# gradslam/gradslam

Hardware: AMD Instinct MI355X
Metric: frames/sec PointFusion 640x480 RGB-D (higher is better)
Workload: dtype f32

## Files before the change

### gradslam_amd/csrc/gs_assoc_dev.h

```cpp
#pragma once
#include "gs_common.h"

struct GsCamera {
  float Ri[9];
  float ti[3];
  float K[12];
};

GS_DEV GsCamera gs_camera(const float* __restrict__ pose16, const float* __restrict__ K16) {
  GsCamera c;
#pragma unroll
  for (int j = 0; j < 3; ++j)
#pragma unroll
    for (int k = 0; k < 3; ++k) c.Ri[3 * j + k] = pose16[4 * k + j];
  const float t0 = pose16[3], t1 = pose16[7], t2 = pose16[11];
#pragma unroll
  for (int j = 0; j < 3; ++j)
    c.ti[j] = gs_dot3_plain(-c.Ri[3 * j], -c.Ri[3 * j + 1], -c.Ri[3 * j + 2], t0, t1, t2);
#pragma unroll
  for (int i = 0; i < 12; ++i) c.K[i] = K16[i];
  return c;
}

GS_DEV bool gs_project_point_hw_q(const GsCamera& c, float p0, float p1, float p2, int H, int W, float u_hi, float v_hi,
                                  int& h_out, int& w_out, float* q) {
  const float q0 = gs_dot3_fma(p0, p1, p2, c.Ri[0], c.Ri[1], c.Ri[2]) + c.ti[0];
  const float q1 = gs_dot3_fma(p0, p1, p2, c.Ri[3], c.Ri[4], c.Ri[5]) + c.ti[1];
  const float q2 = gs_dot3_fma(p0, p1, p2, c.Ri[6], c.Ri[7], c.Ri[8]) + c.ti[2];
  q[0] = q0;
  q[1] = q1;
  q[2] = q2;
  const bool front = q2 > 0.0f;
  float r[3];
#pragma unroll
  for (int j = 0; j < 3; ++j) {
    float acc = c.K[4 * j] * q0;
    acc = acc + c.K[4 * j + 1] * q1;
    acc = acc + c.K[4 * j + 2] * q2;
    acc = acc + c.K[4 * j + 3] * 1.0f;
    r[j] = acc;
  }
  const float zz = (r[2] != 0.0f) ? r[2] : 1.0f;
  const float u = r[0] / zz, v = r[1] / zz;
  const bool in_frame = (u > -1e-3f) && (u < u_hi) && (v > -1e-3f) && (v < v_hi) && front;
  if (!in_frame) return false;
  int wi = (int)__builtin_rintf(u), hi = (int)__builtin_rintf(v);
  wi = wi < 0 ? 0 : (wi > W - 1 ? W - 1 : wi);
  hi = hi < 0 ? 0 : (hi > H - 1 ? H - 1 : hi);
  h_out = hi;
  w_out = wi;
  return true;
}
GS_DEV bool gs_project_point_hw(const GsCamera& c, float p0, float p1, float p2, int H, int W, float u_hi, float v_hi,
                                int& h_out, int& w_out) {
  float q[3];
  return gs_project_point_hw_q(c, p0, p1, p2, H, W, u_hi, v_hi, h_out, w_out, q);
}

GS_DEV int32_t gs_project_point(const GsCamera& c, float p0, float p1, float p2, int H, int W,
                                float u_hi, float v_hi) {
  int h, w;
  return gs_project_point_hw(c, p0, p1, p2, H, W, u_hi, v_hi, h, w) ? (int32_t)(h * W + w) : -1;
}

GS_DEV bool gs_on_lattice(int h, int w, int ds) {
  if ((ds & (ds - 1)) == 0) return ((h | w) & (ds - 1)) == 0;
  return ((unsigned)h % (unsigned)ds == 0u) && ((unsigned)w % (unsigned)ds == 0u);
}

GS_DEV bool gs_is_similar(const float* __restrict__ points, const float* __restrict__ normals,
                          const float* __restrict__ gvertex, const float* __restrict__ gnormal,
                          int64_t n, int64_t p, float dist_th, float dot_th) {
  const float f0 = gvertex[3 * p], f1 = gvertex[3 * p + 1], f2 = gvertex[3 * p + 2];
  const float q0 = points[3 * n], q1 = points[3 * n + 1], q2 = points[3 * n + 2];
  const float dist = gs_norm3(f0 - q0, f1 - q1, f2 - q2);
  const float dot = gs_dot3_plain(gnormal[3 * p], gnormal[3 * p + 1], gnormal[3 * p + 2], normals[3 * n],
                                  normals[3 * n + 1], normals[3 * n + 2]);
  return (dist < dist_th) && (dot > dot_th);
}

GS_DEV bool gs_is_similar_v(const float* __restrict__ points, const float* __restrict__ normals, const float* f,
                            const float* g, int64_t n, float dist_th, float dot_th) {
  const float q0 = points[3 * n], q1 = points[3 * n + 1], q2 = points[3 * n + 2];
  const float dist = gs_norm3(f[0] - q0, f[1] - q1, f[2] - q2);
  const float dot = gs_dot3_plain(g[0], g[1], g[2], normals[3 * n], normals[3 * n + 1], normals[3 * n + 2]);
  return (dist < dist_th) && (dot > dot_th);
}

GS_DEV uint64_t gs_assoc_key(const float* __restrict__ points, const float* __restrict__ ccounts,
                             const float* __restrict__ gvertex, int64_t n, int64_t p) {
  const float inv = 1.0f / (ccounts[n] + 1e-20f);
  const float d0 = points[3 * n] - gvertex[3 * p];
  const float d1 = points[3 * n + 1] - gvertex[3 * p + 1];
  const float d2 = points[3 * n + 2] - gvertex[3 * p + 2];
  float ray = d0 * d0 + d1 * d1;
  ray = ray + d2 * d2;
  return ((uint64_t)__float_as_uint(inv) << 32) | (uint64_t)__float_as_uint(ray);
}
GS_DEV uint64_t gs_assoc_key_v(const float* __restrict__ points, const float* __restrict__ ccounts, const float* f,
                               int64_t n) {
  const float inv = 1.0f / (ccounts[n] + 1e-20f);
  const float d0 = points[3 * n] - f[0];
  const float d1 = points[3 * n + 1] - f[1];
  const float d2 = points[3 * n + 2] - f[2];
  float ray = d0 * d0 + d1 * d1;
  ray = ray + d2 * d2;
  return ((uint64_t)__float_as_uint(inv) << 32) | (uint64_t)__float_as_uint(ray);
}
```

### gradslam_amd/csrc/gs_fuse.hip

```cpp
#include "gs_assoc_dev.h"
#include "gs_compact.h"

__global__ void __launch_bounds__(256) gs_fuse_init_kernel(int32_t* __restrict__ pix_of, int64_t n,
                                                           int32_t* __restrict__ any_flag) {
  const int64_t i = (int64_t)blockIdx.x * 256 + threadIdx.x;
  if (i == 0) *any_flag = 0;
  if (i < n) pix_of[i] = -1;
}

__global__ void __launch_bounds__(256) gs_fuse_scatter_kernel(const int32_t* __restrict__ best_pix,
                                                              int64_t P, GsCount n_map_c,
                                                              int32_t* __restrict__ pix_of,
                                                              int32_t* __restrict__ any_flag) {
  const int64_t p = (int64_t)blockIdx.x * 256 + threadIdx.x;
  if (p >= P) return;
  const int32_t n = best_pix[p];
  if (n >= 0 && n < gs_count(n_map_c)) {
    pix_of[n] = (int32_t)p;
    *any_flag = 1;
  }
}

struct FrameGlobalMaps {
  const float* __restrict__ gvertex;
  const float* __restrict__ gnormal;
  __device__ void operator()(const int64_t p, float* fp, float* fn) const {
#pragma unroll
    for (int k = 0; k < 3; ++k) {
      fp[k] = gvertex[3 * p + k];
      fn[k] = gnormal[3 * p + k];
    }
  }
  __device__ void vertex_of(const int64_t p, float* fp) const {
#pragma unroll
    for (int k = 0; k < 3; ++k) fp[k] = gvertex[3 * p + k];
  }
  __device__ void normal_of(const int64_t p, float* fn) const {
#pragma unroll
    for (int k = 0; k < 3; ++k) fn[k] = gnormal[3 * p + k];
  }
};
struct FrameLocalMaps {
  const float* __restrict__ vertex;
  const float* __restrict__ normal;
  float T[12];
  __device__ void operator()(const int64_t p, float* fp, float* fn) const {
    float v[3], n[3];
#pragma unroll
    for (int k = 0; k < 3; ++k) {
      v[k] = vertex[3 * p + k];
      n[k] = normal[3 * p + k];
    }
    const float validf = v[2] > 0.0f ? 1.0f : 0.0f;
    float g0, g1, g2;
    gs_rigid_fma(T, v[0], v[1], v[2], g0, g1, g2);
    fp[0] = g0 * validf; fp[1] = g1 * validf; fp[2] = g2 * validf;
    fn[0] = gs_dot3_fma(T[0], T[1], T[2], n[0], n[1], n[2]);
    fn[1] = gs_dot3_fma(T[4], T[5], T[6], n[0], n[1], n[2]);
    fn[2] = gs_dot3_fma(T[8], T[9], T[10], n[0], n[1], n[2]);
  }
  __device__ void vertex_of(const int64_t p, float* fp) const {
    float v[3];
#pragma unroll
    for (int k = 0; k < 3; ++k) v[k] = vertex[3 * p + k];
    const float validf = v[2] > 0.0f ? 1.0f : 0.0f;
    float g0, g1, g2;
    gs_rigid_fma(T, v[0], v[1], v[2], g0, g1, g2);
    fp[0] = g0 * validf; fp[1] = g1 * validf; fp[2] = g2 * validf;
  }
  __device__ void normal_of(const int64_t p, float* fn) const {
    float n[3];
#pragma unroll
    for (int k = 0; k < 3; ++k) n[k] = normal[3 * p + k];
    fn[0] = gs_dot3_fma(T[0], T[1], T[2], n[0], n[1], n[2]);
    fn[1] = gs_dot3_fma(T[4], T[5], T[6], n[0], n[1], n[2]);
    fn[2] = gs_dot3_fma(T[8], T[9], T[10], n[0], n[1], n[2]);
  }
};
GS_DEV FrameLocalMaps frame_local_maps(const float* vertex, const float* normal, const float* pose16) {
  FrameLocalMaps f;
  f.vertex = vertex; f.normal = normal;
#pragma unroll
  for (int i = 0; i < 12; ++i) f.T[i] = pose16[i];
  return f;
}

template <class Frame>
GS_DEV void fuse_merge_row(float* __restrict__ points, float* __restrict__ normals, float* __restrict__ colors,
                           float* __restrict__ ccounts, const int64_t n, const int32_t p, const Frame& frame,
                           const float* __restrict__ rgb, const float* __restrict__ alpha) {
  const float a = p >= 0 ? alpha[p] : 0.0f;
  const float cc = ccounts[n];
  float P[3], N[3], C[3], fp[3] = {0.0f, 0.0f, 0.0f}, fn[3] = {0.0f, 0.0f, 0.0f}, fc[3] = {0.0f, 0.0f, 0.0f};
#pragma unroll
  for (int k = 0; k < 3; ++k) {
    P[k] = points[3 * n + k];
    N[k] = normals[3 * n + k];
    C[k] = colors[3 * n + k];
  }
  if (p >= 0) {
    frame((int64_t)p, fp, fn);
#pragma unroll
    for (int k = 0; k < 3; ++k) fc[k] = rgb[3 * (int64_t)p + k];
  }
  const float cc2 = cc + a;
  const float inv = 1.0f / (cc2 == 0.0f ? 1.0f : cc2);
#pragma unroll
  for (int k = 0; k < 3; ++k) {
    P[k] = ((cc * P[k]) + (a * fp[k])) * inv;
    N[k] = ((cc * N[k]) + (a * fn[k])) * inv;
    C[k] = ((cc * C[k]) + (a * fc[k])) * inv;
  }
#pragma unroll
  for (int k = 0; k < 3; ++k) points[3 * n + k] = P[k];
#pragma unroll
  for (int k = 0; k < 3; ++k) normals[3 * n + k] = N[k];
#pragma unroll
  for (int k = 0; k < 3; ++k) colors[3 * n + k] = C[k];
  ccounts[n] = cc2;
}

__global__ void __launch_bounds__(256) gs_fuse_merge_kernel(
    float* __restrict__ points, float* __restrict__ normals, float* __restrict__ colors,
    float* __restrict__ ccounts, GsCount n_map_c, const int32_t* __restrict__ pix_of,
    const int32_t* __restrict__ any_flag, const float* __restrict__ gvertex,
    const float* __restrict__ gnormal, const float* __restrict__ rgb, const float* __restrict__ alpha,
    int renorm_all) {
  const int64_t n = (int64_t)blockIdx.x * 256 + threadIdx.x;
  if (n >= gs_count(n_map_c)) return;
  if (*any_flag == 0 && renorm_all != 2) return;
  const int32_t p = pix_of[n];
  if (p < 0 && !renorm_all) return;
  fuse_merge_row(points, normals, colors, ccounts, n, p, FrameGlobalMaps{gvertex, gnormal}, rgb, alpha);
}

struct PredNewPixel {
  const float* depth;
  const int32_t* best_pix;
  __device__ bool operator()(int64_t p) const {
    return depth[p] > 0.0f && (best_pix == nullptr || best_pix[p] < 0);
  }
};
template <class Frame>
struct EmitAppendT {
  float* points;
  float* normals;
  float* colors;
  float* ccounts;
  GsCount n_map;
  Frame frame;
  const float* rgb;
  const float* alpha;
  __device__ void operator()(int64_t p, int64_t pos) const {
    const int64_t r = gs_count(n_map) + pos;
    float v[3], nn[3] = {0.0f, 0.0f, 0.0f}, c[3] = {0.0f, 0.0f, 0.0f};
    frame.vertex_of(p, v);
    if (normals) frame.normal_of(p, nn);
    if (colors) {
#pragma unroll
      for (int k = 0; k < 3; ++k) c[k] = rgb[3 * p + k];
    }
    const float a = ccounts ? alpha[p] : 0.0f;
#pragma unroll
    for (int k = 0; k < 3; ++k) points[3 * r + k] = v[k];
    if (normals) {
#pragma unroll
      for (int k = 0; k < 3; ++k) normals[3 * r + k] = nn[k];
    }
    if (colors) {
#pragma unroll
      for (int k = 0; k < 3; ++k) colors[3 * r + k] = c[k];
    }
    if (ccounts) ccounts[r] = a;
  }
};
typedef EmitAppendT<FrameGlobalMaps> EmitAppend;

static int fuse_append(float* points, float* normals, float* colors, float* ccounts, GsCount n_map_c,
                       int64_t capacity, const int32_t* best_pix, const float* gvertex, const float* gnormal,
                       const float* rgb, const float* alpha, const float* depth, int H, int W, int renorm_all,
                       int64_t* new_count_out, void* scratch, void* stream) {
  const int64_t n_map_host = n_map_c.host;
  GS_REQUIRE(H > 0 && W > 0 && n_map_host >= 0 && capacity >= n_map_host, "bad sizes");
  GS_REQUIRE(points && normals && colors && ccounts && best_pix && gvertex && gnormal && rgb && alpha &&
                 depth && new_count_out && scratch,
             "NULL pointer");
  hipStream_t st = gs_stream(stream);
  const int64_t P = (int64_t)H * W;
  const int64_t n_map = n_map_host;
  char* base = reinterpret_cast<char*>(scratch) + gs_cp_scratch_bytes(P > n_map ? P : n_map);
  int32_t* any_flag = reinterpret_cast<int32_t*>(base);
  int32_t* pix_of = reinterpret_cast<int32_t*>(base + 256);
  GsProf prof(GS_PROF_FUSE, 88.0 * (double)n_map + 45.0 * (double)P, st);
  if (n_map > 0) {
    hipLaunchKernelGGL(gs_fuse_init_kernel, dim3((unsigned)gs_ceil_div(n_map, 256)), dim3(256), 0, st,
                       pix_of, n_map, any_flag);
    hipLaunchKernelGGL(gs_fuse_scatter_kernel, dim3((unsigned)gs_ceil_div(P, 256)), dim3(256), 0, st,
                       best_pix, P, n_map_c, pix_of, any_flag);
    hipLaunchKernelGGL(gs_fuse_merge_kernel, dim3((unsigned)gs_ceil_div(n_map, 256)), dim3(256), 0, st,
                       points, normals, colors, ccounts, n_map_c, pix_of, any_flag, gvertex, gnormal, rgb,
                       alpha, renorm_all);
    GS_LAUNCH_CHECK();
  }
  EmitAppend emit{points, normals, colors, ccounts, n_map_c, FrameGlobalMaps{gvertex, gnormal}, rgb, alpha};
  return gs_compact(GsCount{P, nullptr}, PredNewPixel{depth, best_pix}, emit, new_count_out, n_map_c, capacity,
                    scratch, st);
}

extern "C" int gs_fuse_append_f32(float* points, float* normals, float* colors, float* ccounts,
                                  int64_t n_map_host, int64_t capacity, const int32_t* best_pix,
                                  const float* gvertex, const float* gnormal, const float* rgb,
                                  const float* alpha, const float* depth, int H, int W, int renorm_all,
                                  int64_t* new_count_out, void* scratch, void* stream) {
  return fuse_append(points, normals, colors, ccounts, GsCount{n_map_host, nullptr}, capacity, best_pix, gvertex,
                     gnormal, rgb, alpha, depth, H, W, renorm_all, new_count_out, scratch, stream);
}
extern "C" int gs_fuse_append_dc_f32(float* points, float* normals, float* colors, float* ccounts,
                                     int64_t n_map_bound, const int64_t* n_map_dev, int64_t capacity,
                                     const int32_t* best_pix, const float* gvertex, const float* gnormal,
                                     const float* rgb, const float* alpha, const float* depth, int H, int W,
                                     int renorm_all, int64_t* new_count_out, void* scratch, void* stream) {
  GS_REQUIRE(n_map_dev && capacity >= n_map_bound + (int64_t)H * W, "device-count fuse needs capacity >= bound + H*W");
  return fuse_append(points, normals, colors, ccounts, GsCount{n_map_bound, n_map_dev}, capacity, best_pix,
                     gvertex, gnormal, rgb, alpha, depth, H, W, renorm_all, new_count_out, scratch, stream);
}

static int append_valid(float* points, float* normals, float* colors, float* ccounts, GsCount n_map_c,
                        int64_t capacity, const float* gvertex, const float* gnormal, const float* rgb,
                        const float* alpha, const float* depth, int H, int W, int64_t* new_count_out,
                        void* scratch, void* stream) {
  GS_REQUIRE(H > 0 && W > 0 && n_map_c.host >= 0 && capacity >= n_map_c.host, "bad sizes");
  GS_REQUIRE(points && gvertex && depth && new_count_out && scratch, "NULL pointer");
  EmitAppend emit{points, gnormal ? normals : nullptr, rgb ? colors : nullptr, alpha ? ccounts : nullptr,
                  n_map_c, FrameGlobalMaps{gvertex, gnormal}, rgb, alpha};
  return gs_compact(GsCount{(int64_t)H * W, nullptr}, PredNewPixel{depth, nullptr}, emit, new_count_out, n_map_c,
                    capacity, scratch, gs_stream(stream));
}
extern "C" int gs_append_valid_f32(float* points, float* normals, float* colors, float* ccounts,
                                   int64_t n_map_host, int64_t capacity, const float* gvertex,
                                   const float* gnormal, const float* rgb, const float* alpha,
                                   const float* depth, int H, int W, int64_t* new_count_out,
                                   void* scratch, void* stream) {
  return append_valid(points, normals, colors, ccounts, GsCount{n_map_host, nullptr}, capacity, gvertex, gnormal,
                      rgb, alpha, depth, H, W, new_count_out, scratch, stream);
}
extern "C" int gs_append_valid_dc_f32(float* points, float* normals, float* colors, float* ccounts,
                                      int64_t n_map_bound, const int64_t* n_map_dev, int64_t capacity,
                                      const float* gvertex, const float* gnormal, const float* rgb,
                                      const float* alpha, const float* depth, int H, int W,
                                      int64_t* new_count_out, void* scratch, void* stream) {
  GS_REQUIRE(n_map_dev && capacity >= n_map_bound + (int64_t)H * W, "device-count append needs capacity >= bound + H*W");
  return append_valid(points, normals, colors, ccounts, GsCount{n_map_bound, n_map_dev}, capacity, gvertex,
                      gnormal, rgb, alpha, depth, H, W, new_count_out, scratch, stream);
}

__global__ void __launch_bounds__(256) gs_fuse_bwd_rows_kernel(
    const float* __restrict__ points, const float* __restrict__ normals, const float* __restrict__ colors,
    const float* __restrict__ ccounts, int64_t n_old, const int32_t* __restrict__ pix_of,
    const int32_t* __restrict__ any_flag, const float* __restrict__ gvertex, const float* __restrict__ gnormal,
    const float* __restrict__ rgb, const float* __restrict__ alpha, int renorm_all,
    const float* __restrict__ P_bar, const float* __restrict__ N_bar, const float* __restrict__ C_bar,
    const float* __restrict__ F_bar, float* __restrict__ oP_bar, float* __restrict__ oN_bar,
    float* __restrict__ oC_bar, float* __restrict__ oF_bar, float* __restrict__ gv_bar, float* __restrict__ gn_bar,
    float* __restrict__ rgb_bar, float* __restrict__ alpha_bar) {
  const int64_t n = (int64_t)blockIdx.x * 256 + threadIdx.x;
  if (n >= n_old) return;
  const int32_t p = (*any_flag != 0) ? pix_of[n] : -1;
  if ((*any_flag == 0 && renorm_all != 2) || (p < 0 && !renorm_all)) {
#pragma unroll
    for (int k = 0; k < 3; ++k) {
      oP_bar[3 * n + k] = P_bar[3 * n + k];
      oN_bar[3 * n + k] = N_bar[3 * n + k];
      oC_bar[3 * n + k] = C_bar[3 * n + k];
    }
    oF_bar[n] = F_bar[n];
    return;
  }
  const double a = p >= 0 ? (double)alpha[p] : 0.0;
  const double cc = (double)ccounts[n];
  const double cc2 = cc + a;
  const double inv = 1.0 / (cc2 == 0.0 ? 1.0 : cc2);
  double inv_bar = 0.0, cc_bar = 0.0, a_bar = 0.0;
  const float* olds[3] = {points, normals, colors};
  const float* frames[3] = {gvertex, gnormal, rgb};
  const float* bars[3] = {P_bar, N_bar, C_bar};
  float* obars[3] = {oP_bar, oN_bar, oC_bar};
  float* fbars[3] = {gv_bar, gn_bar, rgb_bar};
#pragma unroll
  for (int t = 0; t < 3; ++t) {
#pragma unroll
    for (int k = 0; k < 3; ++k) {
      const double x = (double)olds[t][3 * n + k];
      const double f = p >= 0 ? (double)frames[t][3 * (int64_t)p + k] : 0.0;
      const double xb = (double)bars[t][3 * n + k];
      const double ub = xb * inv;
      inv_bar += xb * (cc * x + a * f);
      obars[t][3 * n + k] = (float)(cc * ub);
      if (p >= 0) fbars[t][3 * (int64_t)p + k] = (float)(a * ub);
      cc_bar += x * ub;
      a_bar += f * ub;
    }
  }
  const double cc2_bar = (double)F_bar[n] + (cc2 != 0.0 ? -inv * inv * inv_bar : 0.0);
  oF_bar[n] = (float)(cc_bar + cc2_bar);
  if (p >= 0) alpha_bar[p] = (float)(a_bar + cc2_bar);
}

struct EmitAppendBackward {
  const float* P_bar;
  const float* N_bar;
  const float* C_bar;
  const float* F_bar;
  int64_t n_old;
  float* gv_bar;
  float* gn_bar;
  float* rgb_bar;
  float* alpha_bar;
  __device__ void operator()(int64_t p, int64_t pos) const {
    const int64_t r = n_old + pos;
#pragma unroll
    for (int k = 0; k < 3; ++k) {
      gv_bar[3 * p + k] = P_bar[3 * r + k];
      gn_bar[3 * p + k] = N_bar[3 * r + k];
      rgb_bar[3 * p + k] = C_bar[3 * r + k];
    }
    alpha_bar[p] = F_bar[r];
  }
};

extern "C" int gs_fuse_append_backward_f32(const float* points, const float* normals, const float* colors,
                                           const float* ccounts, int64_t n_old, const int32_t* best_pix,
                                           const float* gvertex, const float* gnormal, const float* rgb,
                                           const float* alpha, const float* depth, int H, int W, int renorm_all,
                                           const float* P_bar, const float* N_bar, const float* C_bar,
                                           const float* F_bar, int64_t n_new, float* old_points_bar,
                                           float* old_normals_bar, float* old_colors_bar, float* old_ccounts_bar,
                                           float* gvertex_bar, float* gnormal_bar, float* rgb_bar, float* alpha_bar,
                                           void* scratch, void* stream) {
  GS_REQUIRE(H > 0 && W > 0 && n_old >= 0 && n_new >= n_old, "bad sizes");
  GS_REQUIRE(best_pix && gvertex && gnormal && rgb && alpha && depth && P_bar && N_bar && C_bar && F_bar && gvertex_bar &&
                 gnormal_bar && rgb_bar && alpha_bar && scratch,
             "NULL pointer");
  hipStream_t st = gs_stream(stream);
  const int64_t P = (int64_t)H * W;
  GS_HIP(hipMemsetAsync(gvertex_bar, 0, 12 * (size_t)P, st));
  GS_HIP(hipMemsetAsync(gnormal_bar, 0, 12 * (size_t)P, st));
  GS_HIP(hipMemsetAsync(rgb_bar, 0, 12 * (size_t)P, st));
  GS_HIP(hipMemsetAsync(alpha_bar, 0, 4 * (size_t)P, st));
  char* base = reinterpret_cast<char*>(scratch) + gs_cp_scratch_bytes(P > n_old ? P : n_old);
  int32_t* any_flag = reinterpret_cast<int32_t*>(base);
  int32_t* pix_of = reinterpret_cast<int32_t*>(base + 256);
  if (n_old > 0) {
    GS_REQUIRE(points && normals && colors && ccounts && old_points_bar && old_normals_bar && old_colors_bar &&
                   old_ccounts_bar,
               "NULL pointer");
    const GsCount n_old_c{n_old, nullptr};
    hipLaunchKernelGGL(gs_fuse_init_kernel, dim3((unsigned)gs_ceil_div(n_old, 256)), dim3(256), 0, st, pix_of, n_old,
                       any_flag);
    hipLaunchKernelGGL(gs_fuse_scatter_kernel, dim3((unsigned)gs_ceil_div(P, 256)), dim3(256), 0, st, best_pix, P,
                       n_old_c, pix_of, any_flag);
    hipLaunchKernelGGL(gs_fuse_bwd_rows_kernel, dim3((unsigned)gs_ceil_div(n_old, 256)), dim3(256), 0, st, points,
                       normals, colors, ccounts, n_old, pix_of, any_flag, gvertex, gnormal, rgb, alpha, renorm_all, P_bar,
                       N_bar, C_bar, F_bar, old_points_bar, old_normals_bar, old_colors_bar, old_ccounts_bar,
                       gvertex_bar, gnormal_bar, rgb_bar, alpha_bar);
    GS_LAUNCH_CHECK();
  }
  EmitAppendBackward emit{P_bar, N_bar, C_bar, F_bar, n_old, gvertex_bar, gnormal_bar, rgb_bar, alpha_bar};
  int64_t* cnt = reinterpret_cast<int64_t*>(base + 128);
  return gs_compact(P, PredNewPixel{depth, best_pix}, emit, cnt, 0, n_new - n_old, scratch, st);
}

constexpr int32_t MU_TIE_MARK = 0x7fffffff;
struct MuSeq {
  float* points; float* normals; float* colors; float* ccounts;
  GsCount n_map;
  int64_t capacity;
  const float* vertex; const float* normal; const float* depth; const float* rgb; const float* alpha;
  const float* pose16; const float* K16;
  float* gvertex; float* gnormal;
  int32_t* best_pix;
  int64_t* new_count_out;
  int32_t* any_flag;
  uint64_t* key_pix;
  int32_t* tile_counts;
  uint64_t* key_pt;
  int32_t* pix;
  int32_t* pix_of;
};
struct MuBatch {
  int B, H, W, renorm_all;
  int64_t P, ntiles;
  float u_hi, v_hi, dist_th, dot_th;
  int32_t* call_flag;
  int zero_call_flag;
  MuSeq s[GS_MAX_BATCH];
};

__global__ void __launch_bounds__(256) gs_mu_pixel_init_kernel(const MuBatch mb) {
  const MuSeq& q = mb.s[blockIdx.x % mb.B];
  const int64_t p = (int64_t)(blockIdx.x / mb.B) * 256 + threadIdx.x;
  if (p == 0) { q.any_flag[0] = 0; q.any_flag[1] = 0; }
  if (blockIdx.x == 0 && threadIdx.x == 0 && mb.zero_call_flag) *mb.call_flag = 0;
  if (p >= mb.P) return;
  float T[12];
#pragma unroll
  for (int i = 0; i < 12; ++i) T[i] = q.pose16[i];
  const float validf = q.depth[p] > 0.0f ? 1.0f : 0.0f;
  float g0, g1, g2;
  gs_rigid_fma(T, q.vertex[3 * p], q.vertex[3 * p + 1], q.vertex[3 * p + 2], g0, g1, g2);
  q.gvertex[3 * p] = g0 * validf;
  q.gvertex[3 * p + 1] = g1 * validf;
  q.gvertex[3 * p + 2] = g2 * validf;
  const float n0 = q.normal[3 * p], n1 = q.normal[3 * p + 1], n2 = q.normal[3 * p + 2];
  q.gnormal[3 * p] = gs_dot3_fma(T[0], T[1], T[2], n0, n1, n2);
  q.gnormal[3 * p + 1] = gs_dot3_fma(T[4], T[5], T[6], n0, n1, n2);
  q.gnormal[3 * p + 2] = gs_dot3_fma(T[8], T[9], T[10], n0, n1, n2);
  q.key_pix[p] = ~0ull;
  q.best_pix[p] = -1;
}

__global__ void __launch_bounds__(256) gs_mu_project_key_kernel(const MuBatch mb) {
  const MuSeq& q = mb.s[blockIdx.x % mb.B];
  const int64_t n = (int64_t)(blockIdx.x / mb.B) * 256 + threadIdx.x;
  if (n >= gs_count(q.n_map)) return;
  const GsCamera c = gs_camera(q.pose16, q.K16);
  const int32_t p = gs_project_point(c, q.points[3 * n], q.points[3 * n + 1], q.points[3 * n + 2], mb.H, mb.W, mb.u_hi,
                                     mb.v_hi);
  int32_t pk = -1;
  if (p >= 0) {
    float fp[3], fn[3];
    if (q.gvertex) FrameGlobalMaps{q.gvertex, q.gnormal}((int64_t)p, fp, fn);
    else frame_local_maps(q.vertex, q.normal, q.pose16)((int64_t)p, fp, fn);
    if (gs_is_similar_v(q.points, q.normals, fp, fn, n, mb.dist_th, mb.dot_th)) {
      const uint64_t k = gs_assoc_key_v(q.points, q.ccounts, fp, n);
      const unsigned long long old = atomicMin(reinterpret_cast<unsigned long long*>(&q.key_pix[p]), (unsigned long long)k);
      if (old == (unsigned long long)k) {
        q.best_pix[p] = MU_TIE_MARK;
        q.any_flag[1] = 1;
      }
      q.key_pt[n] = k;
      pk = p;
    }
  }
  q.pix[n] = pk;
}

GS_DEV void mu_settle_ties(const MuSeq& q, const unsigned blk, const unsigned nblk) {
  if (q.any_flag[1] == 0) return;
  const int64_t n_map = gs_count(q.n_map);
  for (int64_t n = (int64_t)blk * GS_CP_BLOCK + threadIdx.x; n < n_map; n += (int64_t)nblk * GS_CP_BLOCK) {
    const int32_t p = q.pix[n];
    if (p < 0 || q.best_pix[p] == -1) continue;
    if (q.key_pt[n] == q.key_pix[p]) atomicMin(reinterpret_cast<unsigned*>(&q.best_pix[p]), (unsigned)n);
  }
}

__global__ void __launch_bounds__(GS_CP_BLOCK) gs_mu_winner_count_kernel(const MuBatch mb) {
  __shared__ int smem[GS_CP_BLOCK / GS_WAVE + 1];
  const MuSeq& q = mb.s[blockIdx.x % mb.B];
  const unsigned blk = blockIdx.x / mb.B;
  const int64_t base = (int64_t)blk * GS_CP_TILE + (int64_t)threadIdx.x * GS_CP_ITEMS;
  int c = 0;
  uint64_t kk[GS_CP_ITEMS];
  float dd[GS_CP_ITEMS];
#pragma unroll
  for (int i = 0; i < GS_CP_ITEMS; ++i) {
    const int64_t pc = base + i < mb.P ? base + i : mb.P - 1;
    kk[i] = q.key_pix[pc];
    dd[i] = q.depth[pc];
  }
  bool any = false;
#pragma unroll
  for (int i = 0; i < GS_CP_ITEMS; ++i) {
    const int64_t p = base + i;
    if (p < mb.P) {
      const bool matched = kk[i] != ~0ull;
      any = any || matched;
      if (dd[i] > 0.0f && !matched) ++c;
    }
  }
  if (any) {
    q.any_flag[0] = 1;
    *mb.call_flag = 1;
  }
  int total;
  (void)gs_block_excl_scan<GS_CP_BLOCK>(c, smem, &total);
  if (threadIdx.x == 0) q.tile_counts[blk] = total;
  mu_settle_ties(q, blk, gridDim.x / mb.B);
}

GS_DEV void mu_merge_body(const MuBatch& mb, const unsigned bid) {
  const MuSeq& q = mb.s[bid % mb.B];
  const int64_t n = (int64_t)(bid / mb.B) * 256 + threadIdx.x;
  if (n >= gs_count(q.n_map)) return;
  if (*mb.call_flag == 0) return;
  int32_t p = q.pix[n];
  if (p >= 0) {
    bool win = q.key_pt[n] == q.key_pix[p];
    if (win) {
      const int32_t bp = q.best_pix[p];
      win = bp == -1 || bp == (int32_t)n;
      if (win && bp == -1) q.best_pix[p] = (int32_t)n;
    }
    if (!win) p = -1;
  }
  if (p < 0 && !mb.renorm_all) return;
  if (q.gvertex) fuse_merge_row(q.points, q.normals, q.colors, q.ccounts, n, p, FrameGlobalMaps{q.gvertex, q.gnormal}, q.rgb, q.alpha);
  else fuse_merge_row(q.points, q.normals, q.colors, q.ccounts, n, p, frame_local_maps(q.vertex, q.normal, q.pose16), q.rgb, q.alpha);
}

GS_DEV void mu_append_body(const MuBatch& mb, const unsigned bid) {
  __shared__ int smem[GS_CP_BLOCK / GS_WAVE + 1];
  const MuSeq& q = mb.s[bid % mb.B];
  const unsigned blk = bid / mb.B;
  int before = 0, all = 0;
  for (int64_t t = threadIdx.x; t < mb.ntiles; t += GS_CP_BLOCK) {
    const int v = q.tile_counts[t];
    all += v;
    if (t < (int64_t)blk) before += v;
  }
  int tile_prefix, total_new, tile_new;
  (void)gs_block_excl_scan<GS_CP_BLOCK>(before, smem, &tile_prefix);
  (void)gs_block_excl_scan<GS_CP_BLOCK>(all, smem, &total_new);
  const int64_t n_map = gs_count(q.n_map);
  if (blk == 0 && threadIdx.x == 0) q.new_count_out[0] = n_map + total_new;
  const int64_t base = (int64_t)blk * GS_CP_TILE + (int64_t)threadIdx.x * GS_CP_ITEMS;
  bool keep[GS_CP_ITEMS];
  int c = 0;
  {
    uint64_t kk[GS_CP_ITEMS];
    float dd[GS_CP_ITEMS];
#pragma unroll
    for (int i = 0; i < GS_CP_ITEMS; ++i) {
      const int64_t pc = base + i < mb.P ? base + i : mb.P - 1;
      kk[i] = q.key_pix[pc];
      dd[i] = q.depth[pc];
    }
#pragma unroll
    for (int i = 0; i < GS_CP_ITEMS; ++i) {
      keep[i] = base + i < mb.P && dd[i] > 0.0f && kk[i] == ~0ull;
      c += keep[i] ? 1 : 0;
    }
  }
  int w = gs_block_excl_scan<GS_CP_BLOCK>(c, smem, &tile_new);
  __shared__ unsigned short loc_s[GS_CP_TILE];
#pragma unroll
  for (int i = 0; i < GS_CP_ITEMS; ++i) {
    if (keep[i]) loc_s[w++] = (unsigned short)(threadIdx.x * GS_CP_ITEMS + i);
  }
  __syncthreads();
  const int64_t tile_base = (int64_t)blk * GS_CP_TILE;
  if (q.gvertex) {
    const EmitAppend emit{q.points, q.normals, q.colors, q.ccounts, q.n_map, FrameGlobalMaps{q.gvertex, q.gnormal}, q.rgb, q.alpha};
    for (int r = threadIdx.x; r < tile_new; r += GS_CP_BLOCK) {
      const int64_t pos = (int64_t)tile_prefix + r;
      if (n_map + pos < q.capacity) emit(tile_base + loc_s[r], pos);
    }
  } else {
    const EmitAppendT<FrameLocalMaps> emit{q.points, q.normals, q.colors, q.ccounts, q.n_map,
                                           frame_local_maps(q.vertex, q.normal, q.pose16), q.rgb, q.alpha};
    for (int r = threadIdx.x; r < tile_new; r += GS_CP_BLOCK) {
      const int64_t pos = (int64_t)tile_prefix + r;
      if (n_map + pos < q.capacity) emit(tile_base + loc_s[r], pos);
    }
  }
}

static_assert(GS_CP_BLOCK == 256, "merge and append blocks share a launch");
__global__ void __launch_bounds__(256) gs_mu_merge_append_kernel(const MuBatch mb, const unsigned nb_append) {
  if (blockIdx.x < nb_append) mu_append_body(mb, blockIdx.x);
  else mu_merge_body(mb, blockIdx.x - nb_append);
}

extern "C" int64_t gs_update_map_scratch_bytes(int64_t n_map_bound, int H, int W) {
  const int64_t P = (int64_t)H * W;
  return (int64_t)(256 + gs_align(8 * (size_t)P) + gs_align(4 * (size_t)gs_cp_tiles(P)) +
                   gs_align(8 * (size_t)(n_map_bound > 0 ? n_map_bound : 1)) +
                   2 * gs_align(4 * (size_t)(n_map_bound > 0 ? n_map_bound : 1)) + 4096);
}

int32_t* gs_update_map_call_flag(void* scratch0) { return reinterpret_cast<int32_t*>(scratch0) + 32; }
void gs_update_map_tables(void* scratch, int32_t** any_flag, uint64_t** key_pix) {
  *any_flag = reinterpret_cast<int32_t*>(scratch);
  *key_pix = reinterpret_cast<uint64_t*>(reinterpret_cast<char*>(scratch) + 256);
}

static int update_chunk(const gs_update_seq* seqs, int B, int H, int W, float dist_th, float dot_th, int renorm_all,
                        hipStream_t st, int phase, int32_t* call_flag, bool first_chunk, bool tables_ready) {
  MuBatch mb;
  mb.B = B; mb.H = H; mb.W = W; mb.renorm_all = renorm_all;
  mb.call_flag = call_flag; mb.zero_call_flag = first_chunk ? 1 : 0;
  mb.P = (int64_t)H * W;
  mb.ntiles = gs_cp_tiles(mb.P);
  mb.u_hi = (float)((double)W - 0.999); mb.v_hi = (float)((double)H - 0.999);
  mb.dist_th = dist_th; mb.dot_th = dot_th;
  int64_t n_max = 0;
  double bytes_assoc = 0.0, bytes_fuse = 0.0;
  for (int b = 0; b < B; ++b) {
    const gs_update_seq& u = seqs[b];
    const int64_t n_map = u.map.n_bound;
    n_max = n_map > n_max ? n_map : n_max;
    char* q = reinterpret_cast<char*>(u.scratch);
    MuSeq& m = mb.s[b];
    m.points = u.map.points; m.normals = u.map.normals; m.colors = u.map.colors; m.ccounts = u.map.ccounts;
    m.n_map = GsCount{u.map.n_bound, u.map.n_dev};
    m.capacity = u.map.capacity;
    m.vertex = u.vertex; m.normal = u.normal; m.depth = u.depth; m.rgb = u.rgb; m.alpha = u.alpha;
    m.pose16 = u.pose16; m.K16 = u.K16;
    m.gvertex = u.gvertex; m.gnormal = u.gnormal; m.best_pix = u.best_pix; m.new_count_out = u.new_count_out;
    m.any_flag = reinterpret_cast<int32_t*>(q); q += 256;
    m.key_pix = reinterpret_cast<uint64_t*>(q); q += gs_align(8 * (size_t)mb.P);
    m.tile_counts = reinterpret_cast<int32_t*>(q); q += gs_align(4 * (size_t)mb.ntiles);
    m.key_pt = reinterpret_cast<uint64_t*>(q); q += gs_align(8 * (size_t)(n_map > 0 ? n_map : 1));
    m.pix = reinterpret_cast<int32_t*>(q); q += gs_align(4 * (size_t)(n_map > 0 ? n_map : 1));
    m.pix_of = reinterpret_cast<int32_t*>(q);
    bytes_assoc += 72.0 * (double)n_map;
    bytes_fuse += 104.0 * (double)n_map + 49.0 * (double)mb.P;
  }
  const unsigned uB = (unsigned)B;
  const unsigned pb = uB * (unsigned)gs_ceil_div(mb.P, 256), nb = uB * (unsigned)gs_ceil_div(n_max > 0 ? n_max : 1, 256);
  if (phase == 0) {
    if (!tables_ready) {
      GsProf prof(GS_PROF_FRAME, (double)B * (double)mb.P * 64.0, st);
      hipLaunchKernelGGL(gs_mu_pixel_init_kernel, dim3(pb), dim3(256), 0, st, mb);
    }
    if (n_max > 0) {
      GsProf prof(GS_PROF_ASSOC, bytes_assoc, st, 1);
      hipLaunchKernelGGL(gs_mu_project_key_kernel, dim3(nb), dim3(256), 0, st, mb);
    }
    GsProf prof(GS_PROF_FUSE, bytes_fuse / 3.0, st, 1);
    hipLaunchKernelGGL(gs_mu_winner_count_kernel, dim3(uB * (unsigned)mb.ntiles), dim3(GS_CP_BLOCK), 0, st, mb);
  } else {
    GsProf prof(GS_PROF_FUSE, bytes_fuse * (2.0 / 3.0), st, 1);
    const unsigned nb_append = uB * (unsigned)mb.ntiles;
    hipLaunchKernelGGL(gs_mu_merge_append_kernel, dim3(nb_append + (n_max > 0 ? nb : 0u)), dim3(256), 0, st, mb, nb_append);
  }
  GS_LAUNCH_CHECK();
  return GS_OK;
}

int gs_update_map_fusion_batch_impl(const gs_update_seq* seqs_host, int B, int H, int W, float dist_th, float dot_th,
                                    int renorm_all, void* stream, bool tables_ready) {
  GS_REQUIRE(seqs_host && B > 0 && H > 0 && W > 0, "bad arguments");
  GS_REQUIRE((int64_t)H * W < (1ll << 31), "too large for int32 indices");
  for (int b = 0; b < B; ++b) {
    const gs_update_seq& u = seqs_host[b];
    GS_REQUIRE(u.map.n_bound >= 0 && u.map.n_bound < 0x7fffffff, "bad map size");
    GS_REQUIRE(u.map.capacity >= u.map.n_bound + (int64_t)H * W, "capacity must cover n_bound + H*W rows");
    GS_REQUIRE(u.map.points && u.map.normals && u.map.colors && u.map.ccounts && u.vertex && u.normal && u.depth && u.rgb &&
                   u.alpha && u.pose16 && u.K16 && u.best_pix && u.new_count_out && u.scratch,
               "NULL pointer");
    GS_REQUIRE((u.gvertex && u.gnormal) || (tables_ready && !u.gvertex && !u.gnormal), "gvertex / gnormal: both or none");
    GS_REQUIRE(u.new_count_out != u.map.n_dev, "new_count_out must not alias the map's device count");
  }
  hipStream_t st = gs_stream(stream);
  int32_t* call_flag = gs_update_map_call_flag(seqs_host[0].scratch);
  for (int phase = 0; phase < 2; ++phase) {
    for (int c0 = 0; c0 < B; c0 += GS_MAX_BATCH) {
      const int nb = B - c0 < GS_MAX_BATCH ? B - c0 : GS_MAX_BATCH;
      const int rc = update_chunk(seqs_host + c0, nb, H, W, dist_th, dot_th, renorm_all, st, phase, call_flag, c0 == 0,
                                  tables_ready);
      if (rc != GS_OK) return rc;
    }
  }
  return GS_OK;
}

extern "C" int gs_update_map_fusion_batch_f32(const gs_update_seq* seqs_host, int B, int H, int W, float dist_th,
                                              float dot_th, int renorm_all, void* stream) {
  return gs_update_map_fusion_batch_impl(seqs_host, B, H, W, dist_th, dot_th, renorm_all, stream, false);
}

extern "C" int gs_update_map_fusion_dc_f32(float* points, float* normals, float* colors, float* ccounts,
                                           int64_t n_map_bound, const int64_t* n_map_dev, int64_t capacity,
                                           const float* vertex, const float* normal, const float* depth,
                                           const float* rgb, const float* alpha, const float* pose16,
                                           const float* K16, int H, int W, float dist_th, float dot_th,
                                           int renorm_all, float* gvertex, float* gnormal, int32_t* best_pix,
                                           int64_t* new_count_out, void* scratch, void* stream) {
  gs_update_seq u;
  u.map = gs_map_view{points, normals, colors, ccounts, capacity, n_map_bound, n_map_dev};
  u.vertex = vertex; u.normal = normal; u.depth = depth; u.rgb = rgb; u.alpha = alpha;
  u.pose16 = pose16; u.K16 = K16;
  u.gvertex = gvertex; u.gnormal = gnormal; u.best_pix = best_pix; u.new_count_out = new_count_out; u.scratch = scratch;
  return gs_update_map_fusion_batch_f32(&u, 1, H, W, dist_th, dot_th, renorm_all, stream);
}
```

### gradslam_amd/csrc/gs_icp_loop.hip

```cpp
#include <stdlib.h>
#include <string.h>

#include <memory>
#include <mutex>
#include <optional>
#include <type_traits>

#include "gs_env.h"
#include "gs_icp_math.h"
#include "gs_knn.h"
#include "gs_knn_bbox.h"

constexpr int GS_ICP_MAX_ITERS = 1024;
struct GsIcpState {
  IcpSmall s[2];
  float trace[GS_ICP_MAX_ITERS * 12];
};

struct TapePtrs {
  float* src;
  int32_t* idx;
  float* sys;
};
GS_DEV void tape_write_sys(float* __restrict__ sys, int it, const double* S, float damp) {
// ... 873 lines not shown
    if (FULL && out_idx) out_idx[s] = j;
    if (tape_idx) tape_idx[s] = keep ? (int32_t)j : -1;
    if (keep) {
      if (FULL) {
        int q = 0;
#pragma unroll
        for (int i = 0; i < 6; ++i)
#pragma unroll
          for (int k = i; k < 6; ++k) v[q++] = (double)a[i] * (double)a[k];
#pragma unroll
        for (int i = 0; i < 6; ++i) v[21 + i] = (double)a[i] * (double)r;
      }
      v[27] = (double)r * (double)r;
    }
  }
  const int lane = threadIdx.x & 63, wave = threadIdx.x >> 6;
#pragma unroll
  for (int i = FULL ? 0 : 27; i < LIN_NV; ++i) {
    const double sum = gs_wave_sum_f64(v[i]);
    if (lane == 0) red[wave][i] = sum;
  }
  __syncthreads();
  if (threadIdx.x < LIN_NV && (FULL || threadIdx.x == 27)) {
    const int i = threadIdx.x;
    partials[(int64_t)blockIdx.x * LIN_NV + i] = ((red[0][i] + red[1][i]) + red[2][i]) + red[3][i];
  }
}

__global__ void __launch_bounds__(SUM_BLOCK) gs_icp_solve_kernel(const double* __restrict__ partials, int nrows,
                                                                 GsIcpState* __restrict__ st, int it,
                                                                 float* __restrict__ tape_sys) {
  __shared__ double S[32];
  __shared__ double sub[SUM_BLOCK / 32][32];
  __shared__ float xi_s[8];
  icp_sum_rows<SUM_BLOCK>(partials, nrows, S, sub);
  if (threadIdx.x >= GS_WAVE) return;
  gs_solve_spd6_wave(S, st->s[0].damp, xi_s);
  __builtin_amdgcn_wave_barrier();
  if (threadIdx.x != 0) return;
  IcpSmall sm = st->s[0];
  if (tape_sys) tape_write_sys(tape_sys, it, S, sm.damp);
  for (int k = 0; k < 6; ++k) sm.xi[k] = xi_s[k];
  icp_solve_finish(S, sm);
  st->s[0] = sm;
}

__global__ void __launch_bounds__(SUM_BLOCK) gs_icp_update_kernel(const double* __restrict__ partials, int nrows,
                                                                  GsIcpState* __restrict__ st, gs_icp_params prm,
                                                                  int it, const float* __restrict__ compose16,
                                                                  float* __restrict__ out_T16) {
  __shared__ double red[SUM_BLOCK / GS_WAVE];
  const double e1 = icp_sum_col27<SUM_BLOCK>(partials, nrows, red);
  if (threadIdx.x != 0) return;
  IcpSmall sm = st->s[0];
  icp_update_math((float)e1, sm, prm, it < GS_ICP_MAX_ITERS ? st->trace + 12 * it : nullptr);
  st->s[0] = sm;
  if (it == prm.numiters - 1) icp_write_result(sm, compose16, out_T16);
}

GS_DEV IcpSmall icp_state_init(const float* __restrict__ init16, float damp) {
  IcpSmall sm;
  for (int i = 0; i < 16; ++i) {
    sm.T_total[i] = init16[i];
    sm.T_step[i] = init16[i];
    sm.Tr[i] = (i % 5 == 0) ? 1.0f : 0.0f;
  }
  for (int i = 0; i < 8; ++i) sm.xi[i] = 0.0f;
  sm.damp = damp;
  sm.err = 0.0f;
  sm.pad[0] = sm.pad[1] = 0.0f;
  return sm;
}
__global__ void gs_icp_init_kernel(GsIcpState* __restrict__ st, const float* __restrict__ init16, float damp,
                                   int numiters, const float* __restrict__ compose16, float* __restrict__ out_T16) {
  if (threadIdx.x != 0) return;
  const IcpSmall sm = icp_state_init(init16, damp);
  st->s[0] = sm;
  st->s[1] = sm;
  if (numiters == 0) icp_write_result(sm, compose16, out_T16);
}

template <class T>
static T* gs_at(void* base, size_t offset) { return reinterpret_cast<T*>(reinterpret_cast<char*>(base) + offset); }
struct GsTake { size_t end = 0; size_t operator()(size_t n) { end += n; return end - n; } };

constexpr int ICP_ROWRED_DOUBLES = 32;
struct IcpLayout { size_t state, rowred, sync, best, srcA, srcB, partials[2], grid, total; };
static IcpLayout icp_layout(int64_t n_src, int64_t n_tgt) {
  GsTake take;
  IcpLayout L;
  L.state = take(gs_align(sizeof(GsIcpState)));
  L.rowred = take(gs_align(sizeof(double) * ICP_ROWRED_DOUBLES));
  L.sync = L.rowred + sizeof(double) * LIN_NV;
  static_assert(8 * ICP_ROWRED_DOUBLES >= 8 * LIN_NV + 4 * PS_WORDS, "the sync record does not fit behind rowred + LIN_NV");
  L.best = take(gs_align(8 * (size_t)n_src));
  L.srcA = take(gs_align(12 * (size_t)n_src)); L.srcB = take(gs_align(12 * (size_t)n_src));
  for (int k = 0; k < 2; ++k) L.partials[k] = take(gs_align(sizeof(double) * LIN_NV * icp_rows(n_src)));
  L.grid = take(gs_knn_grid_scratch_bytes(n_src, n_tgt));
  L.total = take.end + 4096;
  return L;
}
struct IcpScratch {
  GsIcpState* state;
  double* rowred;
  unsigned* sync;
  unsigned long long* best; float *srcA, *srcB;
  double* partials[2]; void* grid;
};
static IcpScratch icp_carve(void* p, const IcpLayout& L) {
  return IcpScratch{gs_at<GsIcpState>(p, L.state), gs_at<double>(p, L.rowred), gs_at<unsigned>(p, L.sync),
                    gs_at<unsigned long long>(p, L.best), gs_at<float>(p, L.srcA), gs_at<float>(p, L.srcB),
                    {gs_at<double>(p, L.partials[0]), gs_at<double>(p, L.partials[1])}, gs_at<void>(p, L.grid)};
}

extern "C" int64_t gs_icp_scratch_bytes(int64_t n_src, int64_t n_tgt) { return (int64_t)icp_layout(n_src < 1 ? 1 : n_src, n_tgt).total; }

static int icp_tape_finish(void* tape, const GsIcpState* state, int64_t n_src, int numiters, hipStream_t st) {
  GsIcpTape t = gs_icp_tape_carve(tape, n_src, numiters);
  if (numiters > 0)
    GS_HIP(hipMemcpyAsync(t.trace, state->trace, sizeof(float) * 12 * (size_t)numiters, hipMemcpyDeviceToDevice, st));
  return GS_OK;
}

static double icp_alg_bytes(int numiters, int64_t n_slots, int64_t n_queries, int64_t n_binned) {
  const double rows = (double)gs_ceil_div(n_slots, FS_QPB);
  const double full = 12.0 * n_slots + 36.0 * n_queries + 8.0 * LIN_NV * rows + 16.0 * n_binned;
  const double look = 12.0 * n_slots + 24.0 * n_queries + 8.0 * rows + 16.0 * n_binned;
  return (double)numiters * (full + look);
}

struct LocSeq {
  const float* vertex;
  const float* depth;
  const float* pose16;
  float* lattice;
  GsIcpState* state;
  float* out_pose16;
  char* clear_ptr;
  int64_t* n_valid;
  int* far_n;
  int* lstat;
  float4* wl_cq;
  unsigned* sync;
};
struct LocBatch {
  int B, W, ds, Wl;
  int64_t n_lat;
  size_t clear_bytes;
  float damp;
  int numiters;
  int count_valid;
  LocSeq s[GS_MAX_BATCH];
};
constexpr int LP_CLEAR_ITEMS = 8;

GS_DEV void loc_prep_block(const LocBatch& lb, const unsigned bid, const unsigned nb_lat) {
  const LocSeq& q = lb.s[bid % lb.B];
  const unsigned blk = bid / lb.B;
  if (blk < nb_lat) {
    const int64_t e = (int64_t)blk * 256 + threadIdx.x;
    int valid = 0;
    if (e < lb.n_lat) {
      const int64_t p = (e / lb.Wl) * lb.ds * (int64_t)lb.W + (e % lb.Wl) * lb.ds;
      float g0 = __builtin_nanf(""), g1 = g0, g2 = g0;
      if (q.depth[p] > 0.0f) {
        float T[12];
#pragma unroll
        for (int i = 0; i < 12; ++i) T[i] = q.pose16[i];
        gs_rigid_fma(T, q.vertex[3 * p], q.vertex[3 * p + 1], q.vertex[3 * p + 2], g0, g1, g2);
        valid = 1;
      }
      q.lattice[3 * e] = g0; q.lattice[3 * e + 1] = g1; q.lattice[3 * e + 2] = g2;
      if (q.wl_cq) q.wl_cq[e] = make_float4(0.0f, 0.0f, 0.0f, 0.0f);
    }
    const unsigned long long m = lb.count_valid ? __ballot(valid) : 0ull;
    if ((threadIdx.x & 63) == 0 && m) atomicAdd(reinterpret_cast<unsigned long long*>(q.n_valid), (unsigned long long)__popcll(m));
    if (blk == 0 && threadIdx.x == 0) {
      float id[16];
      for (int i = 0; i < 16; ++i) id[i] = (i % 5 == 0) ? 1.0f : 0.0f;
      const IcpSmall sm = icp_state_init(id, lb.damp);
      q.state->s[0] = sm;
      q.state->s[1] = sm;
      if (q.far_n)
        for (int i = 0; i < FS_FAR_PASSES; ++i) q.far_n[i] = 0;
      if (q.lstat)
        for (int i = 0; i < 3 * GL_STAT_LAUNCHES; ++i) q.lstat[i] = 0;
      if (q.sync)
        for (int i = 0; i < PS_WORDS; ++i) q.sync[i] = 0u;
      if (lb.numiters == 0) icp_write_result(sm, q.pose16, q.out_pose16);
    }
    return;
  }
  float4* dst = reinterpret_cast<float4*>(q.clear_ptr);
  const size_t n16 = lb.clear_bytes / 16;
  const size_t base = (size_t)(blk - nb_lat) * 256 * LP_CLEAR_ITEMS + threadIdx.x;
#pragma unroll
  for (int u = 0; u < LP_CLEAR_ITEMS; ++u) {
    const size_t i = base + (size_t)u * 256;
    if (i < n16) dst[i] = make_float4(0.0f, 0.0f, 0.0f, 0.0f);
  }
}
__global__ void __launch_bounds__(256) gs_loc_prep_kernel(const LocBatch lb, unsigned nb_lat) {
  loc_prep_block(lb, blockIdx.x, nb_lat);
}
static_assert(GB_BLOCK == 256, "lattice and bbox blocks share a launch");
__global__ void __launch_bounds__(256) gs_loc_prep_bbox_kernel(const LocBatch lb, const GsGridBatch gb, const unsigned nb_lat,
                                                               const float u_hi, const float v_hi) {
  const unsigned n_prep = (unsigned)lb.B * nb_lat;
  if (blockIdx.x < n_prep) loc_prep_block(lb, blockIdx.x, nb_lat);
  else gridb_bbox_block(gb, blockIdx.x - n_prep, u_hi, v_hi);
}

static int64_t loc_lattice(int H, int W, int ds) { return (int64_t)((H + ds - 1) / ds) * ((W + ds - 1) / ds); }

struct ListMem {
  float4* lq;
  uint32_t* ls;
  int* stat;
};

struct FarMem {
  uint32_t* c;
  float4* cq;
  int* idx;
  int* n;
};

struct FarBuildSeq {
  const float* src;
  const int* idx;
  const int* n;
  const GsGrid* gp;
  const int* cell_start;
  const float4* sorted;
  float* d2prev;
  FarMem m;
};
struct FarBuildBatch {
  int B;
  FarBuildSeq s[GS_MAX_BATCH];
};
constexpr int FAR_BLOCK = 512;
constexpr int FAR_BLOCKS_PER_SEQ = 64;
__global__ void __launch_bounds__(FAR_BLOCK) gs_icp_far_build_kernel(const FarBuildBatch fb) {
  const FarBuildSeq& q = fb.s[blockIdx.x % fb.B];
  const int blk = (int)(blockIdx.x / fb.B);
  const int n = *q.n;
  if (blk >= n) return;
  constexpr int NG = FAR_BLOCK / FS_HG;
  __shared__ float qs[NG][3];
  __shared__ float d1_s[NG];
  __shared__ uint8_t flag_s[NG];
  __shared__ int unres_q[NG], sq_s[NG];
  __shared__ int unres_n;
  __shared__ uint32_t stage_s[NG][GS_FAR_SLOTS + 4];
  const GsGrid g = *q.gp;
  const int grp = threadIdx.x / FS_HG, l16 = threadIdx.x & (FS_HG - 1);
  for (int base = blk; base < n; base += FAR_BLOCKS_PER_SEQ * NG) {
    if (threadIdx.x == 0) unres_n = 0;
    __syncthreads();
    const int e = base + grp * FAR_BLOCKS_PER_SEQ;
    if (e < n) {
      const int sq = q.idx[e];
      const float hx = q.src[3 * (int64_t)sq], hy = q.src[3 * (int64_t)sq + 1], hz = q.src[3 * (int64_t)sq + 2];
      const float4 found = q.m.cq[sq];
      const float d1 = sqrtf(found.x);
      const int kdone = (int)found.y;
      if (kdone >= 0) {
        const float R = far_emit_cube<FS_HG>(g, q.cell_start, q.sorted, hx, hy, hz, l16, d1, kdone, stage_s[grp],
                                             reinterpret_cast<int*>(&stage_s[grp][GS_FAR_SLOTS]));
        for (int u = l16; u < GS_FAR_SLOTS; u += FS_HG) q.m.c[GS_FAR_SLOTS * (int64_t)sq + u] = stage_s[grp][u];
        if (l16 == 0) {
          q.m.cq[sq] = make_float4(hx, hy, hz, R);
          if (R > 0.0f) q.d2prev[sq] = __uint_as_float(__float_as_uint(q.d2prev[sq]) | 0x80000000u);
        }
      } else if (l16 == 0) {
        qs[grp][0] = hx; qs[grp][1] = hy; qs[grp][2] = hz;
        d1_s[grp] = d1;
        sq_s[grp] = sq;
        unres_q[atomicAdd(&unres_n, 1)] = grp;
      }
    }
    __syncthreads();
    const int nun = unres_n;
    for (int u = 0; u < nun; u += FS_BQ) {
      const int nq = nun - u < FS_BQ ? nun - u : FS_BQ;
      block_brute_collect_multi<FAR_BLOCK, FS_BQ>(qs, unres_q + u, nq, q.sorted, q.cell_start[g.ncell], d1_s,
                                                  GS_FAR_RADD * g.c, sq_s, q.m.cq, q.m.c, flag_s);
      if ((int)threadIdx.x < nq) {
        const int gq = unres_q[u + threadIdx.x];
        const int s2 = sq_s[gq];
        if (flag_s[gq]) q.d2prev[s2] = __uint_as_float(__float_as_uint(q.d2prev[s2]) | 0x80000000u);
      }
    }
    __syncthreads();
  }
}

static int64_t loc_rows(const gs_map_view& m) { return m.capacity > m.n_bound ? m.capacity : m.n_bound; }

struct LocLayout {
  int64_t n_lat, rows;
  IcpLayout sc;
  size_t lattice, pix, n_valid, icp, lq, ls, lstat, far_c, far_cq, far_idx, far_n, far_out4, total;
};
static LocLayout loc_layout(int64_t n_lat, int64_t rows) {
  GsTake take;
  LocLayout L;
  L.n_lat = n_lat; L.rows = rows > 0 ? rows : 1;
  L.lattice = take(gs_align(12 * (size_t)n_lat));
  L.pix = take(gs_align(4 * (size_t)L.rows));
  L.n_valid = take(256);
  L.sc = icp_layout(n_lat, L.rows);
  L.icp = take(L.sc.total);
  L.lq = take(gs_align(16 * (size_t)n_lat));
  L.ls = take(gs_align(4 * GL_SLOTS * (size_t)n_lat));
  L.lstat = take(gs_align(4 * 3 * GL_STAT_LAUNCHES));
  L.far_c = take(gs_align(4 * GS_FAR_SLOTS * (size_t)n_lat));
  L.far_cq = take(gs_align(16 * (size_t)n_lat));
  L.far_idx = take(gs_align(4 * FS_FAR_PASSES * (size_t)n_lat));
  L.far_n = take(256);
  L.far_out4 = L.far_n + 4 * 8;
  static_assert(FS_FAR_PASSES <= 8, "the far-list counters run into the result words");
  L.total = take.end;
  return L;
}
static bool loc_lists_fit(const LocLayout& L) { return L.total - (L.icp + L.sc.partials[1]) >= sizeof(double) * LIN_NV * FS_BLOCK; }

extern "C" int64_t gs_localize_scratch_bytes(int H, int W, int ds, int64_t n_map_bound) {
  if (H < 1 || W < 1 || ds < 1) return 0;
  return (int64_t)loc_layout(loc_lattice(H, W, ds), n_map_bound).total;
}

struct LocCarve {
  float* lattice; int32_t* pix; int64_t* n_valid;
  IcpScratch sc; GridMem gm; ListMem lm;
  FarMem fm; int* far_out4;
};
static LocCarve loc_carve(void* p, const LocLayout& L) {
  const IcpScratch sc = icp_carve(gs_at<char>(p, L.icp), L.sc);
  return LocCarve{gs_at<float>(p, L.lattice), gs_at<int32_t>(p, L.pix), gs_at<int64_t>(p, L.n_valid), sc,
                  grid_carve(sc.grid, L.n_lat, L.rows),
                  ListMem{gs_at<float4>(p, L.lq), gs_at<uint32_t>(p, L.ls), gs_at<int>(p, L.lstat)},
                  FarMem{gs_at<uint32_t>(p, L.far_c), gs_at<float4>(p, L.far_cq), gs_at<int>(p, L.far_idx), gs_at<int>(p, L.far_n)},
                  gs_at<int>(p, L.far_out4)};
}
static LocCarve loc_carve_of(const void* scratch, int H, int W, int ds, int64_t map_rows) {
  return loc_carve(const_cast<void*>(scratch), loc_layout(loc_lattice(H, W, ds), map_rows));
}

struct IcpEnginePlan {
  bool far_on, wide_on, lists_on, persist_on;
  bool binned_normals;
  bool reduce_rows;
  int lists_from;
  IcpHalfPlan half;
  int ps_it0, ps_nb, ps_upb;
  float weak_room;
  int lmode(int it, bool look_ahead) const {
    if (!lists_on || it < lists_from) return 0;
    if (it > lists_from) return 2;
    return look_ahead ? (persist_on ? 3 : 1) : 0;
  }
};
static IcpEnginePlan icp_engine_plan(const GsEnv& env, const IcpDevice& dev, int B, int64_t n_lat, int numiters,
                                     const LocLayout* layouts) {
  IcpEnginePlan p;
  const int64_t rows = (int64_t)icp_rows(n_lat);
  p.binned_normals = env.icp_binned_normals; p.weak_room = env.icp_weak_room;
  p.lists_from = env.icp_lists_from >= 0 ? env.icp_lists_from : FS_LISTS_FROM;
  p.reduce_rows = rows > FS_REDUCE_ROWS;
  p.far_on = env.icp_far && numiters > 0;
  p.wide_on = env.icp_wide && !p.far_on && numiters > 0;
  p.ps_upb = (int)gs_ceil_div(rows, PS_CUS_PER_XCD);
  p.ps_nb = (int)gs_ceil_div(rows, p.ps_upb > 0 ? p.ps_upb : 1);
  const bool persist_asked = env.icp_persist && env.icp_lists && !p.far_on && B <= (int)GS_XCDS && p.ps_upb <= PS_UPB &&
                             numiters > p.lists_from + 1 && !env.icp_timeline && !env.icp_lanes_set && dev.ps_fits &&
                             p.binned_normals;
  p.half = icp_half_plan(env, dev.cus, n_lat, B, p.far_on ? 4 : (persist_asked ? 2 : 8));
  p.lists_on = env.icp_lists && !p.far_on && p.half.upb * p.half.G * FS_QPB <= FS_BLOCK;
  for (int b = 0; b < B && p.lists_on; ++b) p.lists_on = loc_lists_fit(layouts[b]);
  p.persist_on = persist_asked && p.half.G == 2 && p.lists_on;
  p.ps_it0 = p.persist_on ? p.lists_from + 1 : numiters;
  return p;
}
static IcpEnginePlan icp_plain_plan(const IcpHalfPlan& half, int64_t n_src, int numiters) {
  IcpEnginePlan p{};
  p.binned_normals = true; p.reduce_rows = icp_rows(n_src) > FS_REDUCE_ROWS;
  p.half = half; p.ps_it0 = numiters;
  return p;
}

struct IcpSolveView {
  const float* src0;
  const float *tgt, *tn; GsCount n_tgt;
  IcpScratch sc; GridMem gm;
  int64_t* out_idx;
  TapePtrs tape;
  IcpHalfLists lists; IcpHalfWide wide; FarMem far;
  const float* compose16; float* out_T16;
  unsigned* sync;
};

static void loc_bind(const gs_localize_seq* seqs, int B, int H, int W, int ds, const gs_icp_params* prm,
                     const IcpEnginePlan& plan, LocCarve* c, LocBatch& lb, GsGridBatch& gb, IcpSolveView* v) {
  lb.B = gb.B = B; lb.W = gb.W = W; gb.H = H; lb.ds = gb.ds = ds;
  lb.Wl = (W + ds - 1) / ds; lb.n_lat = loc_lattice(H, W, ds); lb.damp = prm->damp; lb.numiters = prm->numiters;
  gb.cells_cap = gs_knn_grid_cells_cap(lb.n_lat);
  for (int b = 0; b < B; ++b) {
    const gs_localize_seq& q = seqs[b];
    if (!plan.binned_normals) c[b].gm.sorted_n = nullptr;
    lb.s[b] = LocSeq{q.vertex, q.depth, q.prev_pose16, c[b].lattice, c[b].sc.state, q.out_pose16,
                     reinterpret_cast<char*>(c[b].gm.g), c[b].n_valid, c[b].fm.n, c[b].lm.stat,
                     plan.wide_on ? c[b].fm.cq : nullptr, c[b].sc.sync};
    gb.s[b] = GsGridSeq{q.map.points, GsCount{q.map.n_bound, q.map.n_dev}, c[b].pix, q.prev_pose16, q.K16,
                        plan.binned_normals ? q.map.normals : nullptr, c[b].gm};
    v[b] = IcpSolveView{c[b].lattice, q.map.points, q.map.normals, GsCount{q.map.n_bound, q.map.n_dev}, c[b].sc, c[b].gm,
                        nullptr, TapePtrs{nullptr, nullptr, nullptr},
                        plan.lists_on ? IcpHalfLists{c[b].lm.lq, c[b].lm.ls, c[b].lm.stat, c[b].sc.sync + PS_WEAK}
                                      : IcpHalfLists{nullptr, nullptr, nullptr, nullptr},
                        plan.wide_on ? IcpHalfWide{c[b].fm.cq, c[b].fm.c} : IcpHalfWide{nullptr, nullptr},
                        plan.far_on ? c[b].fm : FarMem{nullptr, nullptr, nullptr, nullptr},
                        q.prev_pose16, q.out_pose16, plan.persist_on ? c[b].sc.sync : nullptr};
  }
  lb.count_valid = g_gs_prof_on ? 1 : 0;
  lb.clear_bytes = gs_knn_grid_clear_bytes(c[0].gm, gb.cells_cap);
}

static int loc_prep(const gs_localize_seq* seqs, const LocBatch& lb, const GsGridBatch& gb, hipStream_t st, bool grid_cleared) {
  const int B = lb.B;
  if (g_gs_prof_on)
    for (int b = 0; b < B; ++b) GS_HIP(hipMemsetAsync(lb.s[b].n_valid, 0, 8, st));
  const unsigned nb_lat = (unsigned)gs_ceil_div(lb.n_lat, 256);
  const unsigned nb_clear = (unsigned)gs_ceil_div((int64_t)(lb.clear_bytes / 16), 256 * LP_CLEAR_ITEMS);
  double bytes = 0.0;
  for (int b = 0; b < B; ++b) bytes += 28.0 * lb.n_lat + 24.0 * seqs[b].map.n_bound + 16.0 * gb.cells_cap;
  GsProf prof(GS_PROF_COMPACT, bytes, st, grid_cleared ? 4 : 5);
  if (grid_cleared) {
    const float u_hi = (float)((double)gb.W - 0.999), v_hi = (float)((double)gb.H - 0.999);
    hipLaunchKernelGGL(gs_loc_prep_bbox_kernel, dim3((unsigned)B * nb_lat + gs_knn_gridb_bbox_blocks(gb)), dim3(256), 0, st,
                       lb, gb, nb_lat, u_hi, v_hi);
    return gs_knn_grid_build_batch(gb, st, true);
  }
  hipLaunchKernelGGL(gs_loc_prep_kernel, dim3((unsigned)B * (nb_lat + nb_clear)), dim3(256), 0, st, lb, nb_lat);
  return gs_knn_grid_build_batch(gb, st);
}

static int loc_prof_bytes(int B, const LocCarve* c, int64_t n_lat, int numiters, hipStream_t st, double* bytes) {
  for (int b = 0; b < B; ++b) {
    unsigned hits = 0; int64_t nv = 0;
    GS_HIP(hipMemcpyAsync(&hits, c[b].gm.bbox + 6, 4, hipMemcpyDeviceToHost, st));
    GS_HIP(hipMemcpyAsync(&nv, c[b].n_valid, 8, hipMemcpyDeviceToHost, st));
    GS_HIP(hipStreamSynchronize(st));
    *bytes += icp_alg_bytes(numiters, n_lat, nv, hits);
  }
  return GS_OK;
}

static const char* icp_params_error(const gs_icp_params* prm) {
  if (!(prm->numiters >= 0 && prm->numiters <= GS_ICP_MAX_ITERS)) return "numiters must be in [0, 1024]";
  return prm->mode == 0 || prm->mode == 1 ? nullptr : "mode must be 0 (ICP) or 1 (gradICP)";
}

struct IcpHalfIo { const double* rows_in; double* rows_out; const IcpSmall* st_in; IcpSmall* st_out; };
static IcpHalfIo icp_half_io(const IcpScratch& sc, int h) {
  return IcpHalfIo{sc.partials[(h + 1) & 1], sc.partials[h & 1], &sc.state->s[h & 1], &sc.state->s[(h + 1) & 1]};
}
static float* icp_cloud(const IcpSolveView& v, int it, int64_t n_src) {
  return v.tape.src ? v.tape.src + (size_t)it * 3 * (size_t)n_src : ((it & 1) ? v.sc.srcB : v.sc.srcA);
}
static int32_t* icp_tape_idx(const IcpSolveView& v, int it, int look_ahead, int64_t n_src) {
  return v.tape.idx ? v.tape.idx + ((size_t)it * 2 + look_ahead) * (size_t)n_src : nullptr;
}

static void loc_half_iterations(const IcpSolveView* v, int B, const IcpEnginePlan& plan, GsCount n_src_c,
                                const gs_icp_params* prm, hipStream_t st, bool prof_rows) {
  const int64_t n_src = n_src_c.host;
  IcpHalfBatch hb;
  hb.B = B; hb.weak_room = plan.weak_room;
  for (int b = 0; b < B; ++b) { hb.w[b] = v[b].wide; hb.l[b] = v[b].lists; }
  for (int it = 0; it < plan.ps_it0; ++it) {
    int h = 2 * it;
    for (int b = 0; b < B; ++b) {
      const IcpSolveView& q = v[b];
      const IcpHalfIo io = icp_half_io(q.sc, h);
      hb.s[b] = IcpHalfSeq{it == 0 ? q.src0 : icp_cloud(q, it - 1, n_src), icp_cloud(q, it, n_src), q.tgt, q.tn, q.n_tgt, q.gm.g,
                           q.gm.cell_start, q.gm.sorted, q.gm.sorted_n, reinterpret_cast<float*>(q.sc.best),
                           io.rows_in, io.rows_out, io.st_in, io.st_out, q.sc.state->trace, q.out_idx,
                           icp_tape_idx(q, it, 0, n_src), nullptr, q.far.cq, q.far.c, q.far.idx, q.far.n};
    }
    icp_half_launch<true>(plan.half, hb, n_src_c, prm, it, 0, st, plan.lmode(it, false));
    if (plan.far_on && fs_far_pass(it) >= 0) {
      const int fp = fs_far_pass(it);
      FarBuildBatch fbb; fbb.B = B;
      for (int b = 0; b < B; ++b)
        fbb.s[b] = FarBuildSeq{icp_cloud(v[b], it, n_src), v[b].far.idx + (int64_t)fp * n_src, v[b].far.n + fp,
                               v[b].gm.g, v[b].gm.cell_start, v[b].gm.sorted, reinterpret_cast<float*>(v[b].sc.best), v[b].far};
      hipLaunchKernelGGL(gs_icp_far_build_kernel, dim3((unsigned)B * FAR_BLOCKS_PER_SEQ), dim3(FAR_BLOCK), 0, st, fbb);
    }
    ++h;
    if (plan.reduce_rows) {
      std::optional<GsProf> prof;
      if (prof_rows) prof.emplace(GS_PROF_SOLVE, 1.0, st);
      IcpRowsBatch rb; rb.B = B;
      for (int b = 0; b < B; ++b) { rb.in[b] = icp_half_io(v[b].sc, h).rows_in; rb.out[b] = v[b].sc.rowred; }
      hipLaunchKernelGGL(gs_icp_reduce_rows_batch_kernel, dim3((unsigned)B), dim3(FS_BLOCK), 0, st, rb, n_src_c);
    }
    for (int b = 0; b < B; ++b) {
      const IcpSolveView& q = v[b];
      const IcpHalfIo io = icp_half_io(q.sc, h);
      IcpHalfSeq& u = hb.s[b];
      u.src_in = icp_cloud(q, it, n_src); u.src_out = nullptr;
      u.partials_in = plan.reduce_rows ? q.sc.rowred : io.rows_in; u.partials_out = io.rows_out;
      u.st_in = io.st_in; u.st_out = io.st_out;
      u.out_idx = nullptr; u.tape_idx = icp_tape_idx(q, it, 1, n_src); u.tape_sys = q.tape.sys;
    }
    icp_half_launch<false>(plan.half, hb, n_src_c, prm, it, plan.reduce_rows ? 1 : 0, st, plan.lmode(it, true));
  }
}

static void loc_persist(const IcpSolveView* v, int B, const IcpEnginePlan& plan, int64_t n_lat, const gs_icp_params* prm,
                        hipStream_t st) {
  IcpPersistBatch pb;
  pb.B = B; pb.nb = plan.ps_nb; pb.upb = plan.ps_upb; pb.h0 = 2 * plan.ps_it0; pb.tl_h = 0; pb.timeline = nullptr;
  for (int b = 0; b < B; ++b) {
    const IcpSolveView& q = v[b];
    const IcpScratch& sc = q.sc; const GridMem& gm = q.gm;
    pb.s[b] = IcpPersistSeq{icp_cloud(q, plan.ps_it0 - 1, n_lat), q.n_tgt, gm.g, gm.cell_start,
                            gm.sorted, gm.sorted_n, {sc.partials[0], sc.partials[1]}, sc.state, q.lists.lq, q.lists.ls,
                            q.lists.lstat, q.wide.cq, q.wide.c, sc.sync};
  }
#ifdef GS_ICP_TIMELINE
  ps_tl_arm(pb, prm->numiters, st);
#endif
  hipLaunchKernelGGL(gs_icp_persist_kernel, dim3(GS_XCDS * PS_CUS_PER_XCD), dim3(PS_BLOCK), 0, st, pb, n_lat, prm->dist_thresh, *prm);
#ifdef GS_ICP_TIMELINE
  ps_tl_dump(pb, st);
#endif
}

static void loc_finish(const IcpSolveView* v, int B, const IcpEnginePlan& plan, GsCount n_src_c, const gs_icp_params* prm,
                       hipStream_t st) {
  const int h = 2 * prm->numiters;
  GsProf prof(GS_PROF_SOLVE, 1.0, st);
  IcpFinishBatch fb;
  fb.B = B; fb.nb = plan.persist_on ? plan.ps_nb : 0; fb.h0 = plan.persist_on ? 2 * plan.ps_it0 : 0;
  for (int b = 0; b < B; ++b) {
    fb.partials_in[b] = icp_half_io(v[b].sc, h).rows_in;
    fb.st[b] = v[b].sc.state; fb.compose16[b] = v[b].compose16; fb.out_T16[b] = v[b].out_T16; fb.sync[b] = v[b].sync;
  }
  hipLaunchKernelGGL(gs_icp_finish_batch_kernel, dim3((unsigned)B), dim3(FS_BLOCK), 0, st, fb, n_src_c, h & 1, *prm);
}

static int icp_run(const float* src, int64_t n_src, const float* tgt, const float* tgt_normals,
                   int64_t n_tgt, const float* init16, const float* compose16,
                   const gs_icp_params* prm, float* out_T16, int64_t* out_idx, void* icp_scratch,
                   void* tape, void* stream, const int64_t* n_src_dev = nullptr,
                   const int64_t* n_tgt_dev = nullptr, GsTargetFilter flt = GsTargetFilter{nullptr, 1, 1}) {
  GS_REQUIRE(prm, "params_host must not be NULL");
  GS_REQUIRE(n_src > 0 && n_tgt > 0, "empty point set");
  GS_REQUIRE(n_tgt < 0x7fffffffll && n_src < 0x7fffffffll, "too many points");
  GS_REQUIRE(src && tgt && tgt_normals && init16 && out_T16 && icp_scratch, "NULL pointer");
  GS_REQUIRE(!icp_params_error(prm), icp_params_error(prm));
  hipStream_t st = gs_stream(stream);
  IcpScratch sc = icp_carve(icp_scratch, icp_layout(n_src, n_tgt));
  hipLaunchKernelGGL(gs_icp_init_kernel, dim3(1), dim3(64), 0, st, sc.state, init16, prm->damp, prm->numiters,
                     compose16, out_T16);
  const bool dev_counts = n_src_dev || n_tgt_dev || flt.pix;
  const bool use_grid = prm->numiters > 0 && (dev_counts || (!gs_env().knn_brute && gs_knn_use_grid(n_src, n_tgt)));
  const GsCount n_src_c{n_src, n_src_dev}, n_tgt_c{n_tgt, n_tgt_dev};
  TapePtrs tp = {nullptr, nullptr, nullptr};
  if (tape) {
    GsIcpTape t = gs_icp_tape_carve(tape, n_src, prm->numiters);
    tp.src = t.src; tp.idx = t.idx; tp.sys = t.sys;
  }
  const IcpSolveView v{src, tgt, tgt_normals, n_tgt_c, sc, grid_carve(sc.grid, n_src, n_tgt), out_idx, tp,
                       IcpHalfLists{nullptr, nullptr, nullptr, nullptr}, IcpHalfWide{nullptr, nullptr},
                       FarMem{nullptr, nullptr, nullptr, nullptr}, compose16, out_T16, nullptr};
  auto cloud = [&](int it) { return icp_cloud(v, it, n_src); };
  auto tidx = [&](int it, int which) { return icp_tape_idx(v, it, which, n_src); };

  if (use_grid) {
    int rc = gs_knn_grid_build(tgt, n_tgt_c, n_src, sc.grid, st, flt, tgt_normals);
    if (rc != GS_OK) return rc;
    double prof_bytes = 0.0;
    if (g_gs_prof_on) {
      int64_t n_binned = n_tgt;
      if (flt.pix) {
        unsigned hits = 0;
        GS_HIP(hipMemcpyAsync(&hits, v.gm.bbox + 6, 4, hipMemcpyDeviceToHost, st));
        GS_HIP(hipStreamSynchronize(st));
        n_binned = hits;
      }
      prof_bytes = icp_alg_bytes(prm->numiters, n_src, n_src, n_binned);
    }
    const IcpEnginePlan plan = icp_plain_plan(icp_half_plan(gs_env(), icp_device().cus, n_src, 1), n_src, prm->numiters);
    {
      GsProf prof(GS_PROF_ICP_FUSED, prof_bytes, st, 2 * prm->numiters);
      loc_half_iterations(&v, 1, plan, n_src_c, prm, st, true);
    }
    loc_finish(&v, 1, plan, n_src_c, prm, st);
    GS_LAUNCH_CHECK();
    if (tape) return icp_tape_finish(tape, sc.state, n_src, prm->numiters, st);
    return GS_OK;
  }

  GS_HIP(hipMemsetAsync(sc.best, 0xff, 8 * (size_t)n_src, st));
  const int nblk = (int)gs_ceil_div(n_src, LIN_BLOCK);
  double* partials = sc.partials[0];
  const float* cur_in = src;
  for (int it = 0; it < prm->numiters; ++it) {
    float* cur = cloud(it);
    gs_knn_brute_launch(cur_in, sc.state->s[0].T_step, cur, n_src, tgt, n_tgt, sc.best, st);
    {
      GsProf prof(GS_PROF_LINEARIZE, 44.0 * (double)n_src, st);
      hipLaunchKernelGGL((gs_icp_linearize_kernel<true>), dim3(nblk), dim3(LIN_BLOCK), 0, st, cur, nullptr, n_src,
                         tgt, tgt_normals, n_tgt, sc.best, prm->dist_thresh, partials, out_idx, tidx(it, 0));
    }
    {
      GsProf prof(GS_PROF_SOLVE, 1.0, st);
      hipLaunchKernelGGL(gs_icp_solve_kernel, dim3(1), dim3(SUM_BLOCK), 0, st, partials, nblk, sc.state, it, tp.sys);
    }
    gs_knn_brute_launch(cur, sc.state->s[0].Tr, nullptr, n_src, tgt, n_tgt, sc.best, st);
    {
      GsProf prof(GS_PROF_LINEARIZE, 44.0 * (double)n_src, st);
      hipLaunchKernelGGL((gs_icp_linearize_kernel<false>), dim3(nblk), dim3(LIN_BLOCK), 0, st, cur,
                         sc.state->s[0].Tr, n_src, tgt, tgt_normals, n_tgt, sc.best, prm->dist_thresh, partials,
                         nullptr, tidx(it, 1));
    }
    {
      GsProf prof(GS_PROF_SOLVE, 1.0, st);
      hipLaunchKernelGGL(gs_icp_update_kernel, dim3(1), dim3(SUM_BLOCK), 0, st, partials, nblk, sc.state, *prm, it,
                         compose16, out_T16);
    }
    cur_in = cur;
  }
  GS_LAUNCH_CHECK();
  if (tape) return icp_tape_finish(tape, sc.state, n_src, prm->numiters, st);
  return GS_OK;
}

extern "C" int gs_icp_f32(const float* src, int64_t n_src, const float* tgt, const float* tgt_normals,
                          int64_t n_tgt, const float* init16, const float* compose16,
                          const gs_icp_params* prm, float* out_T16, int64_t* out_idx, void* icp_scratch,
                          void* stream) {
  return icp_run(src, n_src, tgt, tgt_normals, n_tgt, init16, compose16, prm, out_T16, out_idx, icp_scratch, nullptr,
                 stream);
}

extern "C" int gs_icp_dc_f32(const float* src, int64_t n_src_bound, const int64_t* n_src_dev, const float* tgt,
                             const float* tgt_normals, int64_t n_tgt_bound, const int64_t* n_tgt_dev,
                             const float* init16, const float* compose16, const gs_icp_params* prm, float* out_T16,
                             int64_t* out_idx, void* icp_scratch, void* stream) {
  return icp_run(src, n_src_bound, tgt, tgt_normals, n_tgt_bound, init16, compose16, prm, out_T16, out_idx,
                 icp_scratch, nullptr, stream, n_src_dev, n_tgt_dev);
}

extern "C" int gs_icp_map_dc_f32(const float* src, int64_t n_src_bound, const int64_t* n_src_dev,
                                 const float* map_points, const float* map_normals, const int32_t* pix,
                                 int64_t n_map_bound, const int64_t* n_map_dev, int W, int ds, const float* init16,
                                 const float* compose16, const gs_icp_params* prm, float* out_T16,
                                 void* icp_scratch, void* stream) {
  GS_REQUIRE(pix && W > 0 && ds > 0, "bad target filter");
  return icp_run(src, n_src_bound, map_points, map_normals, n_map_bound, init16, compose16, prm, out_T16, nullptr,
                 icp_scratch, nullptr, stream, n_src_dev, n_map_dev, GsTargetFilter{pix, W, ds});
}

static int localize_chunk(const gs_localize_seq* seqs, int B, int H, int W, int ds, const gs_icp_params* prm,
                          hipStream_t st, bool grid_cleared) {
  const int64_t n_lat = loc_lattice(H, W, ds);
  LocLayout layouts[GS_MAX_BATCH]; LocCarve c[GS_MAX_BATCH];
  for (int b = 0; b < B; ++b) {
    layouts[b] = loc_layout(n_lat, loc_rows(seqs[b].map));
    c[b] = loc_carve(seqs[b].scratch, layouts[b]);
  }
  const IcpEnginePlan plan = icp_engine_plan(gs_env(), icp_device(), B, n_lat, prm->numiters, layouts);
  LocBatch lb; GsGridBatch gb; IcpSolveView v[GS_MAX_BATCH];
  loc_bind(seqs, B, H, W, ds, prm, plan, c, lb, gb, v);
  int rc = loc_prep(seqs, lb, gb, st, grid_cleared);
  if (rc != GS_OK) return rc;
  if (prm->numiters == 0) { GS_LAUNCH_CHECK(); return GS_OK; }
  double prof_bytes = 0.0;
  if (g_gs_prof_on && (rc = loc_prof_bytes(B, c, n_lat, prm->numiters, st, &prof_bytes)) != GS_OK) return rc;
  {
    GsProf prof(GS_PROF_ICP_FUSED, prof_bytes, st, 2 * prm->numiters);
    loc_half_iterations(v, B, plan, GsCount{n_lat, nullptr}, prm, st, false);
    if (plan.persist_on) loc_persist(v, B, plan, n_lat, prm, st);
  }
  loc_finish(v, B, plan, GsCount{n_lat, nullptr}, prm, st);
  GS_LAUNCH_CHECK();
  return GS_OK;
}

static int localize_batch(const gs_localize_seq* seqs_host, int B, int H, int W, int ds, const gs_icp_params* prm,
                          void* stream, bool grid_cleared) {
  GS_REQUIRE(seqs_host && prm && B > 0 && H > 0 && W > 0 && ds > 0, "bad arguments");
  GS_REQUIRE(!icp_params_error(prm), icp_params_error(prm));
  GS_REQUIRE((int64_t)H * W < (1ll << 31), "image too large for int32 pixel ids");
  for (int b = 0; b < B; ++b) {
    const gs_localize_seq& q = seqs_host[b];
    GS_REQUIRE(q.vertex && q.depth && q.K16 && q.prev_pose16 && q.out_pose16 && q.scratch, "NULL pointer");
    GS_REQUIRE(q.map.points && q.map.normals && q.map.n_bound > 0 && q.map.n_bound < 0x7fffffffll,
               "every sequence needs a non-empty map (points + normals)");
    GS_REQUIRE(q.map.capacity <= 0 || q.map.n_bound <= q.map.capacity, "map.n_bound exceeds map.capacity");
  }
  hipStream_t st = gs_stream(stream);
  for (int c0 = 0; c0 < B; c0 += GS_MAX_BATCH) {
    const int nb = B - c0 < GS_MAX_BATCH ? B - c0 : GS_MAX_BATCH;
    const int rc = localize_chunk(seqs_host + c0, nb, H, W, ds, prm, st, grid_cleared);
    if (rc != GS_OK) return rc;
  }
  return GS_OK;
}
extern "C" int gs_localize_batch_f32(const gs_localize_seq* seqs_host, int B, int H, int W, int ds,
                                     const gs_icp_params* prm, void* stream) {
  return localize_batch(seqs_host, B, H, W, ds, prm, stream, false);
}

__global__ void __launch_bounds__(256) gs_far_stats_kernel(const int* __restrict__ far_idx, const int* __restrict__ far_n,
                                                          const float* __restrict__ d2prev, const float4* __restrict__ far_cq,
                                                          int64_t n_lat, int* __restrict__ out4) {
  const int n0 = far_n[0], n = n0 < 0 ? 0 : (n0 > (int)n_lat ? (int)n_lat : n0);
  if (blockIdx.x == 0 && threadIdx.x == 0) { out4[0] = n; out4[2] = far_n[1]; }
  int c = 0, built = 0;
  for (int i = blockIdx.x * 256 + threadIdx.x; i < n; i += gridDim.x * 256) {
    const int s = far_idx[i];
    if (s < 0 || s >= (int)n_lat) continue;
    c += (__float_as_uint(d2prev[s]) >> 31) ? 1 : 0;
    built += far_cq[s].w > 0.0f ? 1 : 0;
  }
  if (c) atomicAdd(&out4[1], c);
  if (built) atomicAdd(&out4[3], built);
}
extern "C" int gs_localize_far_stats_i64(const void* scratch, int H, int W, int ds, int64_t map_rows, int64_t* out4_host,
                                         void* stream) {
  GS_REQUIRE(scratch && out4_host && H > 0 && W > 0 && ds > 0 && map_rows > 0, "bad arguments");
  const int64_t n_lat = loc_lattice(H, W, ds);
  const LocCarve cv = loc_carve_of(scratch, H, W, ds, map_rows);
  const FarMem& fm = cv.fm; hipStream_t st = gs_stream(stream);
  int* out4 = cv.far_out4;
  GS_HIP(hipMemsetAsync(out4, 0, 16, st));
  hipLaunchKernelGGL(gs_far_stats_kernel, dim3(64), dim3(256), 0, st, fm.idx, fm.n, reinterpret_cast<const float*>(cv.sc.best),
                     fm.cq, n_lat, out4);
  int h[4] = {0, 0, 0, 0};
  GsGrid g;
  GS_HIP(hipMemcpyAsync(h, out4, 16, hipMemcpyDeviceToHost, st));
  GS_HIP(hipMemcpyAsync(&g, cv.gm.g, sizeof(g), hipMemcpyDeviceToHost, st));
  GS_HIP(hipStreamSynchronize(st));
  for (int i = 0; i < 4; ++i) out4_host[i] = h[i];
  if (gs_env().debug_grid)
    fprintf(stderr, "grid: box (%.3f %.3f %.3f)-(%.3f %.3f %.3f) c %.4f cells %d x %d x %d = %d\n", g.ox, g.oy, g.oz, g.mx,
            g.my, g.mz, g.c, g.nx, g.ny, g.nz, g.ncell);
  return GS_OK;
}

extern "C" int gs_localize_list_stats_i64(const void* scratch, int H, int W, int ds, int64_t map_rows, int64_t* out192_host,
                                          void* stream) {
  GS_REQUIRE(scratch && out192_host && H > 0 && W > 0 && ds > 0 && map_rows > 0, "bad arguments");
  const ListMem lm = loc_carve_of(scratch, H, W, ds, map_rows).lm;
  int h[3 * GL_STAT_LAUNCHES];
  hipStream_t st = gs_stream(stream);
  GS_HIP(hipMemcpyAsync(h, lm.stat, sizeof(h), hipMemcpyDeviceToHost, st));
  GS_HIP(hipStreamSynchronize(st));
  for (int i = 0; i < 3 * GL_STAT_LAUNCHES; ++i) out192_host[i] = h[i];
  return GS_OK;
}

extern "C" int gs_localize_solve_stats_i64(const void* scratch, int H, int W, int ds, int64_t map_rows, int64_t* out8_host,
                                           void* stream) {
  GS_REQUIRE(scratch && out8_host && H > 0 && W > 0 && ds > 0 && map_rows > 0, "bad arguments");
  const LocCarve cv = loc_carve_of(scratch, H, W, ds, map_rows);
  unsigned h[PS_WORDS];
  hipStream_t st = gs_stream(stream);
  GS_HIP(hipMemcpyAsync(h, cv.sc.sync, sizeof(h), hipMemcpyDeviceToHost, st));
  GS_HIP(hipStreamSynchronize(st));
  static_assert(PS_WORDS == 8, "out8");
  for (int i = 0; i < PS_WORDS; ++i) out8_host[i] = h[i];
  return GS_OK;
}

extern "C" int gs_pointfusion_step_batch_f32(const gs_step_seq* seqs_host, int B, int H, int W, int ds,
                                             const gs_icp_params* prm, float two_sigma_sq, float dist_th, float dot_th,
                                             int renorm_all, void* stream) {
  GS_REQUIRE(seqs_host && prm && B > 0 && H > 0 && W > 0 && ds > 0, "bad arguments");
  const int64_t P = (int64_t)H * W;
  const gs_step_seq& s0 = seqs_host[0];
  const int64_t dstride = B > 1 ? seqs_host[1].depth - s0.depth : P;
  for (int b = 0; b < B; ++b) {
    const gs_step_seq& q = seqs_host[b];
    GS_REQUIRE(q.depth && q.rgb && q.K16 && q.prev_pose16 && q.out_pose16 && q.vertex && q.normal && q.alpha &&
                   q.best_pix && q.new_count_out && q.loc_scratch && q.upd_scratch, "NULL pointer");
    GS_REQUIRE((q.gvertex != nullptr) == (q.gnormal != nullptr) && (q.gvertex != nullptr) == (s0.gvertex != nullptr),
               "gvertex / gnormal: both or none, the same choice for every sequence");
    GS_REQUIRE(q.out_pose16 != q.prev_pose16, "out_pose16 must not alias prev_pose16");
    GS_REQUIRE(q.vertex == s0.vertex + 3 * P * b && q.normal == s0.normal + 3 * P * b && q.alpha == s0.alpha + P * b,
               "vertex / normal / alpha of the batch must be dense");
    GS_REQUIRE(q.depth == s0.depth + dstride * b && q.K16 == s0.K16 + 16 * (int64_t)b, "depth / K16 must be equally strided");
  }
  GS_REQUIRE(dstride >= P || B == 1, "overlapping depth images");
  const bool implicit_global = s0.gvertex == nullptr;
  std::unique_ptr<gs_update_seq[]> us(new gs_update_seq[B]);
  for (int c0 = 0; c0 < B; c0 += GS_MAX_BATCH) {
    const int nb = B - c0 < GS_MAX_BATCH ? B - c0 : GS_MAX_BATCH;
    const gs_step_seq* sq = seqs_host + c0;
    gs_localize_seq ls[GS_MAX_BATCH];
    for (int b = 0; b < nb; ++b) {
      const gs_step_seq& q = sq[b];
      ls[b].vertex = q.vertex; ls[b].depth = q.depth; ls[b].K16 = q.K16; ls[b].prev_pose16 = q.prev_pose16;
      ls[b].map = q.map; ls[b].out_pose16 = q.out_pose16; ls[b].scratch = q.loc_scratch;
      gs_update_seq& u = us[c0 + b];
      u.map = q.map; u.vertex = q.vertex; u.normal = q.normal; u.depth = q.depth; u.rgb = q.rgb;
      u.alpha = q.alpha; u.pose16 = q.out_pose16; u.K16 = q.K16; u.gvertex = q.gvertex;
      u.gnormal = q.gnormal; u.best_pix = q.best_pix; u.new_count_out = q.new_count_out;
      u.scratch = q.upd_scratch;
    }
    GsClearJob job;
    job.n = nb;
    for (int b = 0; b < nb; ++b) {
      GS_REQUIRE(ls[b].map.points && ls[b].map.n_bound > 0, "every sequence needs a non-empty map");
      const LocCarve cv = loc_carve_of(ls[b].scratch, H, W, ds, loc_rows(ls[b].map));
      job.ptr[b] = reinterpret_cast<char*>(cv.gm.g);
      if (b == 0) job.bytes = gs_knn_grid_clear_bytes(cv.gm, gs_knn_grid_cells_cap(loc_lattice(H, W, ds)));
    }
    GsPixelTables tabs{};
    tabs.n = implicit_global ? nb : 0;
    tabs.call_flag = c0 == 0 ? gs_update_map_call_flag(seqs_host[0].upd_scratch) : nullptr;
    for (int b = 0; b < tabs.n; ++b) {
      gs_update_map_tables(sq[b].upd_scratch, &tabs.any_flag[b], &tabs.key_pix[b]);
      tabs.best_pix[b] = sq[b].best_pix;
    }
    int rc = gs_frame_maps_batch_clear(sq[0].depth, dstride, P, sq[0].K16, nb, 1, H, W, two_sigma_sq, sq[0].vertex,
                                       sq[0].normal, sq[0].alpha, &job, stream, &tabs);
    if (rc != GS_OK) return rc;
    rc = localize_batch(ls, nb, H, W, ds, prm, stream, true);
    if (rc != GS_OK) return rc;
  }
  return gs_update_map_fusion_batch_impl(us.get(), B, H, W, dist_th, dot_th, renorm_all, stream, implicit_global);
}

extern "C" int64_t gs_icp_tape_bytes(int64_t n_src, int numiters) { return (int64_t)gs_icp_tape_size(n_src, numiters); }

extern "C" int gs_icp_tape_f32(const float* src, int64_t n_src, const float* tgt, const float* tgt_normals,
                               int64_t n_tgt, const float* init16, const float* compose16,
                               const gs_icp_params* prm, float* out_T16, int64_t* out_idx, void* icp_scratch,
                               void* tape, void* stream) {
  GS_REQUIRE(tape, "tape must not be NULL");
  return icp_run(src, n_src, tgt, tgt_normals, n_tgt, init16, compose16, prm, out_T16, out_idx, icp_scratch, tape,
                 stream);
}

extern "C" int gs_icp_trace_f32(const void* icp_scratch, int numiters, float* trace_out, void* stream) {
  GS_REQUIRE(icp_scratch && trace_out && numiters >= 0 && numiters <= GS_ICP_MAX_ITERS, "bad arguments");
  const GsIcpState* st = reinterpret_cast<const GsIcpState*>(icp_scratch);
  GS_HIP(hipMemcpyAsync(trace_out, st->trace, sizeof(float) * 12 * (size_t)numiters, hipMemcpyDeviceToDevice,
                        gs_stream(stream)));
  return GS_OK;
}
```

### gradslam_amd/csrc/gs_knn.h

```cpp
#pragma once
#include "gs_common.h"

GS_DEV unsigned long long knn_pack(float d, uint32_t idx) {
  return ((unsigned long long)__float_as_uint(d) << 32) | (unsigned long long)idx;
}

int gs_knn_brute_launch(const float* src_in, const float* Tapply, float* src_out, int64_t n_src,
                        const float* tgt, int64_t n_tgt, unsigned long long* best, hipStream_t st);

constexpr int GS_GRID_MAXCELL = 1 << 22;
constexpr int GS_GRID_RINGS = 3;
constexpr int GS_GRID_TILE = 1024;

struct GsGrid {
  float ox, oy, oz;
  float mx, my, mz;
  float c, inv_c;
  int nx, ny, nz, ncell;
};

struct GsTargetFilter {
  const int32_t* pix;
  int W, ds;
};
GS_DEV bool gs_is_target(const GsTargetFilter& f, int64_t n) {
  if (!f.pix) return true;
  const int32_t p = f.pix[n];
  return p >= 0 && ((p / f.W) % f.ds == 0) && ((p % f.W) % f.ds == 0);
}

struct GridMem {
  GsGrid* g;
  unsigned* bbox;
  int* unres_count;
  int* cell_count;
  int* cell_start;
  int* tile_sums;
  float4* sorted;
  float4* sorted_n;
  float4* tlist;
  int* unres_list;
};

static inline GridMem grid_carve(void* scratch, int64_t n_src, int64_t n_tgt) {
  char* p = reinterpret_cast<char*>(scratch);
  GridMem m;
  m.g = reinterpret_cast<GsGrid*>(p); p += 128;
  m.bbox = reinterpret_cast<unsigned*>(p); p += 128;
  m.unres_count = reinterpret_cast<int*>(p); p += 256;
  m.tile_sums = reinterpret_cast<int*>(p); p += gs_align(4 * (size_t)(GS_GRID_MAXCELL / GS_GRID_TILE + 2));
  m.cell_count = reinterpret_cast<int*>(p); p += gs_align(4 * (size_t)(GS_GRID_MAXCELL + 1));
  m.cell_start = reinterpret_cast<int*>(p); p += gs_align(4 * (size_t)(GS_GRID_MAXCELL + 1));
  m.sorted = reinterpret_cast<float4*>(p); p += gs_align(16 * (size_t)(n_tgt > 0 ? n_tgt : 1));
  m.sorted_n = reinterpret_cast<float4*>(p); p += gs_align(16 * (size_t)(n_tgt > 0 ? n_tgt : 1));
  m.tlist = reinterpret_cast<float4*>(p); p += gs_align(16 * (size_t)(n_tgt > 0 ? n_tgt : 1));
  m.unres_list = reinterpret_cast<int*>(p);
  (void)n_src;
  return m;
}

size_t gs_knn_grid_scratch_bytes(int64_t n_src, int64_t n_tgt);

struct GsGridSeq {
  const float* tgt;
  GsCount n_tgt;
  int32_t* pix;
  const float* pose16;
  const float* K16;
  const float* nrm;
  GridMem m;
};
struct GsGridBatch {
  int B, H, W, ds;
  int cells_cap;
  GsGridSeq s[GS_MAX_BATCH];
};
int gs_knn_grid_cells_cap(int64_t n_src);
size_t gs_knn_grid_clear_bytes(const GridMem& m, int cells_cap);
int gs_knn_grid_build_batch(const GsGridBatch& gb, hipStream_t st, bool bbox_done = false);

int gs_knn_grid_build(const float* tgt, GsCount n_tgt, int64_t n_src, void* grid_scratch, hipStream_t st,
                      GsTargetFilter filter = GsTargetFilter{nullptr, 1, 1}, const float* nrm = nullptr);
int gs_knn_grid_query(const float* src_in, const float* Tapply, float* src_out, int64_t n_src,
                      const float* tgt, int64_t n_tgt, unsigned long long* best, void* grid_scratch,
                      hipStream_t st);
static inline bool gs_knn_use_grid(int64_t n_src, int64_t n_tgt) { return n_tgt >= 2048 && n_src >= 256; }

GS_DEV int grid_axis(float v, float o, float inv_c, int n) {
  const float f = (v - o) * inv_c;
  return f >= 0.0f ? (f < (float)n ? (int)f : n - 1) : 0;
}
GS_DEV int grid_cell(const GsGrid& g, float x, float y, float z) {
  const int ix = grid_axis(x, g.ox, g.inv_c, g.nx);
  const int iy = grid_axis(y, g.oy, g.inv_c, g.ny);
  const int iz = grid_axis(z, g.oz, g.inv_c, g.nz);
  return (iz * g.ny + iy) * g.nx + ix;
}

constexpr int GQ_G = 8;
constexpr int GL_RING_NF = 2;

GS_DEV unsigned long long grid_key(float qx, float qy, float qz, const float4 p) {
  const float dx = qx - p.x, dy = qy - p.y, dz = qz - p.z;
  float d = dx * dx;
  d = gs_fma(dy, dy, d);
  d = gs_fma(dz, dz, d);
  return d == d ? knn_pack(d, (uint32_t)__float_as_int(p.w)) : ~0ull;
}

template <int G>
GS_DEV unsigned long long grid_group_min(unsigned long long key) {
#pragma unroll
  for (int d = G / 2; d > 0; d >>= 1) {
    const unsigned long long o = __shfl_xor(key, d, G);
    key = o < key ? o : key;
  }
  return key;
}

struct GsQueryCell {
  float px, py, pz;
  int cx, cy, cz;
};
GS_DEV GsQueryCell grid_query_cell(const GsGrid& g, float qx, float qy, float qz) {
  GsQueryCell c;
  c.px = qx < g.ox ? g.ox : (qx > g.mx ? g.mx : qx);
  c.py = qy < g.oy ? g.oy : (qy > g.my ? g.my : qy);
  c.pz = qz < g.oz ? g.oz : (qz > g.mz ? g.mz : qz);
  c.cx = grid_axis(c.px, g.ox, g.inv_c, g.nx); c.cy = grid_axis(c.py, g.oy, g.inv_c, g.ny);
  c.cz = grid_axis(c.pz, g.oz, g.inv_c, g.nz);
  return c;
}

template <int G>
GS_DEV unsigned long long grid_search_stage0(const GsGrid& g, const int* __restrict__ cell_start,
                                             const float4* __restrict__ sorted, float qx, float qy, float qz, int lane,
                                             bool* resolved, int* win, const float rball = __builtin_inff()) {
  const GsQueryCell qc = grid_query_cell(g, qx, qy, qz);
  const float px = qc.px, py = qc.py, pz = qc.pz;
  const int cx = qc.cx, cy = qc.cy, cz = qc.cz;
  unsigned long long key = ~0ull;
  int bt = -1;
  const float fx = (px - g.ox) * g.inv_c - (float)cx, fy = (py - g.oy) * g.inv_c - (float)cy,
              fz = (pz - g.oz) * g.inv_c - (float)cz;
  const int x0 = (fx < 0.5f) ? cx - 1 : cx, y0 = (fy < 0.5f) ? cy - 1 : cy, z0 = (fz < 0.5f) ? cz - 1 : cz;
  const float BIG = 3.0e38f;
  const float ax = fminf(x0 >= 1 ? fx + (float)(cx - x0) : BIG, x0 + 2 < g.nx ? (float)(x0 + 2 - cx) - fx : BIG);
  const float ay = fminf(y0 >= 1 ? fy + (float)(cy - y0) : BIG, y0 + 2 < g.ny ? (float)(y0 + 2 - cy) - fy : BIG);
  const float az = fminf(z0 >= 1 ? fz + (float)(cz - z0) : BIG, z0 + 2 < g.nz ? (float)(z0 + 2 - cz) - fz : BIG);
  const float amin = fminf(ax, fminf(ay, az));
  const float rc = rball * g.inv_c * 1.0001f + 0.002f;
  const bool prune = rc < amin - 0.001f;
  bool ulx = true, uhx = true, uly = true, uhy = true, ulz = true, uhz = true;
  if (prune) {
    const float tx = fx + (float)(cx - x0), ty = fy + (float)(cy - y0), tz = fz + (float)(cz - z0);
    ulx = tx - rc < 1.0f; uhx = tx + rc >= 1.0f;
    uly = ty - rc < 1.0f; uhy = ty + rc >= 1.0f;
    ulz = tz - rc < 1.0f; uhz = tz + rc >= 1.0f;
  }
  int sb0 = 0, sb1 = 0, sb2 = 0, sb3 = 0, e1 = 0, e2 = 0, e3 = 0, total = 0;
  {
    const int xa = (x0 >= 0 && ulx) ? x0 : x0 + 1, xb = (x0 + 1 < g.nx && uhx) ? x0 + 1 : x0;
    const bool zl = z0 >= 0 && ulz, zh = z0 + 1 < g.nz && uhz, yl = y0 >= 0 && uly, yh = y0 + 1 < g.ny && uhy;
    const int r0 = (z0 * g.ny + y0) * g.nx, r1 = r0 + g.nx, r2 = r0 + g.ny * g.nx, r3 = r2 + g.nx;
    int se0 = 0, se1 = 0, se2 = 0, se3 = 0;
    if (zl && yl) { sb0 = cell_start[r0 + xa]; se0 = cell_start[r0 + xb + 1]; }
    if (zl && yh) { sb1 = cell_start[r1 + xa]; se1 = cell_start[r1 + xb + 1]; }
    if (zh && yl) { sb2 = cell_start[r2 + xa]; se2 = cell_start[r2 + xb + 1]; }
    if (zh && yh) { sb3 = cell_start[r3 + xa]; se3 = cell_start[r3 + xb + 1]; }
    e1 = se0 - sb0;
    e2 = e1 + (se1 - sb1);
    e3 = e2 + (se2 - sb2);
    total = e3 + (se3 - sb3);
  }
  for (int t0 = lane; t0 < total; t0 += 4 * G) {
    float4 p[4];
    bool in[4];
#pragma unroll
    for (int u = 0; u < 4; ++u) {
      const int t = t0 + u * G;
      in[u] = t < total;
      const int tt = in[u] ? t : 0;
      const int ix = tt < e1 ? sb0 + tt : (tt < e2 ? sb1 + (tt - e1) : (tt < e3 ? sb2 + (tt - e2) : sb3 + (tt - e3)));
      p[u] = sorted[ix];
    }
#pragma unroll
    for (int u = 0; u < 4; ++u) {
      const unsigned long long k2 = in[u] ? grid_key(qx, qy, qz, p[u]) : ~0ull;
      const bool better = k2 < key;
      key = better ? k2 : key;
      bt = better ? t0 + u * G : bt;
    }
  }
  {
    const unsigned long long kmin = grid_group_min<G>(key);
    const int bs = bt < e1 ? sb0 + bt : (bt < e2 ? sb1 + (bt - e1) : (bt < e3 ? sb2 + (bt - e2) : sb3 + (bt - e3)));
    *win = (key == kmin && bt >= 0) ? bs : -1;
    key = kmin;
  }
  const float rb = (amin < 1.0e30f) ? (amin - 0.001f) * g.c : BIG;
  const float bd = __uint_as_float((uint32_t)(key >> 32));
  *resolved = prune ? (bd == bd) : (rb > 0.0f && (rb >= 1.0e30f ? bd == bd : bd <= rb * rb));
  return key;
}

template <int G>
GS_DEV unsigned long long grid_search_rings(const GsGrid& g, const int* __restrict__ cell_start,
                                            const float4* __restrict__ sorted, float qx, float qy, float qz, int lane,
                                            unsigned long long key, bool* resolved, int* win,
                                            const int kmax = GS_GRID_RINGS, int* kdone = nullptr) {
  const GsQueryCell qc = grid_query_cell(g, qx, qy, qz);
  bool done = false;
  int bs = -1;
  int k = 1;
  for (; k <= kmax && !done; ++k) {
    const int side = 2 * k + 1, nrow = side * side;
    const int xa = qc.cx - k < 0 ? 0 : qc.cx - k, xb = qc.cx + k >= g.nx ? g.nx - 1 : qc.cx + k;
    for (int r = lane; r < nrow; r += G) {
      const int zz = qc.cz + r / side - k, yy = qc.cy + r % side - k;
      if (zz < 0 || zz >= g.nz || yy < 0 || yy >= g.ny) continue;
      const int row = (zz * g.ny + yy) * g.nx;
      const int je = cell_start[row + xb + 1];
      for (int j = cell_start[row + xa]; j < je; j += GL_RING_NF) {
        float4 p[GL_RING_NF];
#pragma unroll
        for (int u = 0; u < GL_RING_NF; ++u) p[u] = sorted[j + u < je ? j + u : je - 1];
#pragma unroll
        for (int u = 0; u < GL_RING_NF; ++u) {
          const unsigned long long k2 = j + u < je ? grid_key(qx, qy, qz, p[u]) : ~0ull;
          if (k2 < key) { key = k2; bs = j + u; }
        }
      }
    }
    {
      const unsigned long long own = key;
      key = grid_group_min<G>(key);
      if (own != key) bs = -1;
    }
    const float rb = (float)k * g.c * 0.999f;
    const float bd = __uint_as_float((uint32_t)(key >> 32));
    done = bd <= rb * rb;
  }
  *resolved = done;
  *win = bs;
  if (kdone) *kdone = k - 1;
  return key;
}

constexpr int GS_FAR_SLOTS = 64;
constexpr float GS_FAR_RADD = 1.0f;

template <int G>
GS_DEV unsigned long long far_list_search(const float4 c0R, const uint32_t* __restrict__ slots,
                                          const float4* __restrict__ sorted, float qx, float qy, float qz, int lane,
                                          bool* proven, int* win) {
  static_assert(GS_FAR_SLOTS == 4 * G, "four list entries per lane");
  const uint4 sl = reinterpret_cast<const uint4*>(slots)[lane];
  const uint32_t s4[4] = {sl.x, sl.y, sl.z, sl.w};
  float4 a[4];
#pragma unroll
  for (int u = 0; u < 4; ++u) a[u] = sorted[s4[u] != ~0u ? s4[u] : 0u];
  unsigned long long k = ~0ull;
  int bs = -1;
#pragma unroll
  for (int u = 0; u < 4; ++u) {
    const unsigned long long k2 = s4[u] != ~0u ? grid_key(qx, qy, qz, a[u]) : ~0ull;
    if (k2 < k) { k = k2; bs = (int)s4[u]; }
  }
  const unsigned long long kmin = grid_group_min<G>(k);
  *win = (k == kmin) ? bs : -1;
  const float bd = __uint_as_float((uint32_t)(kmin >> 32));
  const float ex = qx - c0R.x, ey = qy - c0R.y, ez = qz - c0R.z;
  const float delta = sqrtf(ex * ex + ey * ey + ez * ez);
  *proven = sqrtf(bd) + delta < c0R.w * 0.9999f;
  return kmin;
}

template <int G>
GS_DEV unsigned long long wide_list_search(const float4 c0R, const uint32_t* __restrict__ slots,
                                           const float4* __restrict__ sorted, float qx, float qy, float qz, int lane,
                                           bool* proven, int* win) {
  static_assert(GS_FAR_SLOTS == 4 * G, "four list entries per lane");
  unsigned long long k = ~0ull;
  int bs = -1;
#pragma unroll
  for (int h = 0; h < 2; ++h) {
    const uint2 sl = reinterpret_cast<const uint2*>(slots)[2 * lane + h];
    const float4 a0 = sorted[sl.x != ~0u ? sl.x : 0u], a1 = sorted[sl.y != ~0u ? sl.y : 0u];
    const unsigned long long k0 = sl.x != ~0u ? grid_key(qx, qy, qz, a0) : ~0ull;
    const unsigned long long k1 = sl.y != ~0u ? grid_key(qx, qy, qz, a1) : ~0ull;
    if (k0 < k) { k = k0; bs = (int)sl.x; }
    if (k1 < k) { k = k1; bs = (int)sl.y; }
  }
  const unsigned long long kmin = grid_group_min<G>(k);
  *win = (k == kmin) ? bs : -1;
  const float bd = __uint_as_float((uint32_t)(kmin >> 32));
  const float ex = qx - c0R.x, ey = qy - c0R.y, ez = qz - c0R.z;
  const float delta = sqrtf(ex * ex + ey * ey + ez * ez);
  *proven = sqrtf(bd) + delta < c0R.w * 0.9999f;
  return kmin;
}

template <int G>
GS_DEV float far_emit_cube(const GsGrid& g, const int* __restrict__ cell_start, const float4* __restrict__ sorted,
                           float qx, float qy, float qz, int lane, const float d1, const int kdone, uint32_t* stage,
                           int* stage_n) {
  const GsQueryCell qc = grid_query_cell(g, qx, qy, qz);
  float radd = GS_FAR_RADD * g.c, R = 0.0f;
  const int kE = (d1 + radd > (float)kdone * g.c * 0.999f) ? kdone + 1 : kdone;
  const int xa = qc.cx - kE < 0 ? 0 : qc.cx - kE, xb = qc.cx + kE >= g.nx ? g.nx - 1 : qc.cx + kE;
  const int side = 2 * kE + 1, nrow = side * side;
  const float rcube = (float)kE * g.c * 0.999f;
  for (int attempt = 0; attempt < 3; ++attempt, radd *= 0.5f) {
    float Rt = d1 + radd;
    Rt = Rt < rcube ? Rt : rcube;
    const float R2 = Rt * Rt;
    if (lane == 0) *stage_n = 0;
    for (int u = lane; u < GS_FAR_SLOTS; u += G) stage[u] = ~0u;
    __builtin_amdgcn_fence(__ATOMIC_RELEASE, "wavefront");
    __builtin_amdgcn_wave_barrier();
    for (int r = lane; r < nrow; r += G) {
      const int zz = qc.cz + r / side - kE, yy = qc.cy + r % side - kE;
      if (zz < 0 || zz >= g.nz || yy < 0 || yy >= g.ny) continue;
      const int row = (zz * g.ny + yy) * g.nx;
      const int je = cell_start[row + xb + 1];
      for (int j = cell_start[row + xa]; j < je; ++j) {
        const float4 c = sorted[j];
        const float dx = qx - c.x, dy = qy - c.y, dz = qz - c.z;
        float d = dx * dx;
        d = gs_fma(dy, dy, d);
        d = gs_fma(dz, dz, d);
        if (d < R2) {
          const int pos = atomicAdd(stage_n, 1);
          if (pos < GS_FAR_SLOTS) stage[pos] = (uint32_t)j;
        }
      }
    }
    __builtin_amdgcn_fence(__ATOMIC_ACQ_REL, "wavefront");
    __builtin_amdgcn_wave_barrier();
    const int n = *stage_n;
    __builtin_amdgcn_wave_barrier();
    if (n <= GS_FAR_SLOTS) { R = Rt; break; }
  }
  return R;
}

constexpr int GL_SLOTS = 8;
constexpr int GL_STAT_LAUNCHES = 64;
constexpr float GL_MIN_ROOM = 0.1f;
template <int G> constexpr int gl_k() { return G == 2 ? 2 : 1; }

template <int KT>
struct GlTop {
  float d[KT + 1];
  int s[KT];
};
template <int KT>
GS_DEV void gl_top_reset(GlTop<KT>& t) {
#pragma unroll
  for (int k = 0; k <= KT; ++k) t.d[k] = __builtin_inff();
#pragma unroll
  for (int k = 0; k < KT; ++k) t.s[k] = -1;
}
template <int KT>
GS_DEV void gl_top_push(GlTop<KT>& t, const float d, const int slot) {
#pragma unroll
  for (int k = KT; k >= 0; --k) {
    const bool before_prev = k > 0 && d < t.d[k - 1];
    const bool before_this = d < t.d[k];
    if (k < KT) t.s[k] = before_prev ? t.s[k - 1] : (before_this ? slot : t.s[k]);
    t.d[k] = before_prev ? t.d[k - 1] : (before_this ? d : t.d[k]);
  }
}
template <int G>
GS_DEV float gl_group_minf(float v) {
#pragma unroll
  for (int d = G / 2; d > 0; d >>= 1) {
    const float o = __shfl_xor(v, d, G);
    v = o < v ? o : v;
  }
  return v;
}

template <int G, int KT, int NFI = (G >= 16 ? 1 : 4)>
GS_DEV unsigned long long grid_search_stage0_top(const GsGrid& g, const int* __restrict__ cell_start,
// ... 400 lines not shown
```

### gradslam_amd/csrc/gs_knn.hip

```cpp
#include "gs_knn.h"

#include <stdlib.h>

#include "gs_assoc_dev.h"
#include "gs_env.h"
#include "gs_knn_bbox.h"

constexpr int KNN_BLOCK = 256;
constexpr int KNN_TCHUNK = 512;

template <bool LISTED, int KNN_SPT>
__global__ void __launch_bounds__(KNN_BLOCK) gs_knn1_kernel(
    const float* __restrict__ src_in, const float* __restrict__ Tapply, float* __restrict__ src_out,
    int64_t n_src, const float* __restrict__ tgt, int64_t n_tgt, unsigned long long* __restrict__ best,
    const int* __restrict__ list, const int* __restrict__ count) {
  constexpr int KNN_STILE = KNN_BLOCK * KNN_SPT;
  __shared__ float4 tl[KNN_TCHUNK];
  const int64_t n_q = LISTED ? (int64_t)(*count) : n_src;
  if (LISTED && n_q == 0) return;
  const int64_t j0 = (int64_t)blockIdx.y * KNN_TCHUNK;
  const int cnt = (int)((n_tgt - j0) < KNN_TCHUNK ? (n_tgt - j0) : KNN_TCHUNK);
  if (cnt <= 0) return;
  for (int i = threadIdx.x; i < cnt; i += KNN_BLOCK) {
    const float* t = tgt + 3 * (j0 + i);
    tl[i] = make_float4(t[0], t[1], t[2], 0.0f);
  }
  float T[12];
  if (Tapply) {
#pragma unroll
    for (int i = 0; i < 12; ++i) T[i] = Tapply[i];
  }
  __syncthreads();
  for (int64_t tile = blockIdx.x; tile * KNN_STILE < n_q; tile += gridDim.x) {
    float sx[KNN_SPT], sy[KNN_SPT], sz[KNN_SPT], bd[KNN_SPT];
    int bi[KNN_SPT];
    int64_t sidx[KNN_SPT];
#pragma unroll
    for (int k = 0; k < KNN_SPT; ++k) {
      const int64_t q = tile * KNN_STILE + k * KNN_BLOCK + threadIdx.x;
      int64_t s = -1;
      if (q < n_q) s = LISTED ? (int64_t)list[q] : q;
      float p0 = 0.0f, p1 = 0.0f, p2 = 0.0f;
      if (s >= 0) {
        p0 = src_in[3 * s];
        p1 = src_in[3 * s + 1];
        p2 = src_in[3 * s + 2];
        if (Tapply) {
          float q0, q1, q2;
          gs_rigid_fma(T, p0, p1, p2, q0, q1, q2);
          p0 = q0; p1 = q1; p2 = q2;
        }
        if (!LISTED && src_out && blockIdx.y == 0) {
          src_out[3 * s] = p0;
          src_out[3 * s + 1] = p1;
          src_out[3 * s + 2] = p2;
        }
      }
      sidx[k] = s;
      sx[k] = p0; sy[k] = p1; sz[k] = p2;
      bd[k] = __builtin_inff();
      bi[k] = 0;
    }
#pragma unroll 4
    for (int j = 0; j < cnt; ++j) {
      const float4 t = tl[j];
#pragma unroll
      for (int k = 0; k < KNN_SPT; ++k) {
        const float dx = sx[k] - t.x, dy = sy[k] - t.y, dz = sz[k] - t.z;
        float d = dx * dx;
        d = gs_fma(dy, dy, d);
        d = gs_fma(dz, dz, d);
        const bool lt = d < bd[k];
        bd[k] = lt ? d : bd[k];
        bi[k] = lt ? j : bi[k];
      }
    }
#pragma unroll
    for (int k = 0; k < KNN_SPT; ++k)
      if (sidx[k] >= 0) atomicMin(&best[sidx[k]], knn_pack(bd[k], (uint32_t)(j0 + bi[k])));
    if (!LISTED) break;
  }
}

int gs_knn_brute_launch(const float* src_in, const float* Tapply, float* src_out, int64_t n_src,
                        const float* tgt, int64_t n_tgt, unsigned long long* best, hipStream_t st) {
  const int spt_env = gs_env().knn_spt;
  const int spt = spt_env == 4 || spt_env == 8 ? spt_env : (n_src * n_tgt >= (int64_t)1 << 27 ? 8 : 4);
  GsProf prof(GS_PROF_KNN, (double)n_src * (double)n_tgt, st);
  if (spt == 8) {
    dim3 grid((unsigned)gs_ceil_div(n_src, KNN_BLOCK * 8), (unsigned)gs_ceil_div(n_tgt, KNN_TCHUNK));
    hipLaunchKernelGGL((gs_knn1_kernel<false, 8>), grid, dim3(KNN_BLOCK), 0, st, src_in, Tapply, src_out, n_src, tgt,
                       n_tgt, best, nullptr, nullptr);
  } else {
    dim3 grid((unsigned)gs_ceil_div(n_src, KNN_BLOCK * 4), (unsigned)gs_ceil_div(n_tgt, KNN_TCHUNK));
    hipLaunchKernelGGL((gs_knn1_kernel<false, 4>), grid, dim3(KNN_BLOCK), 0, st, src_in, Tapply, src_out, n_src, tgt,
                       n_tgt, best, nullptr, nullptr);
  }
  return GS_OK;
}

size_t gs_knn_grid_scratch_bytes(int64_t n_src, int64_t n_tgt) {
  return 512 + 2 * gs_align(4 * (size_t)(GS_GRID_MAXCELL + 1)) + gs_align(4 * (size_t)(GS_GRID_MAXCELL / GS_GRID_TILE + 2)) +
         3 * gs_align(16 * (size_t)(n_tgt > 0 ? n_tgt : 1)) + gs_align(4 * (size_t)(n_src > 0 ? n_src : 1)) + 256;
}

__global__ void __launch_bounds__(GB_BLOCK) gs_grid_bbox_kernel(const float* __restrict__ tgt, GsCount n_tgt_c,
                                                                 const GsTargetFilter flt,
                                                                 unsigned* __restrict__ bbox,
                                                                 int* __restrict__ unres_count,
                                                                 float4* __restrict__ tlist) {
  grid_bbox_body(tgt, gs_count(n_tgt_c), flt, nullptr, 0, 0.0f, 0.0f, nullptr, bbox, unres_count, tlist, blockIdx.x);
}

GS_DEV GsGrid grid_from_bbox(const unsigned* __restrict__ bbox, int64_t n_tgt, int cells_cap) {
  float o[3], m[3];
#pragma unroll
  for (int k = 0; k < 3; ++k) {
    const unsigned cl = bbox[k], ch = bbox[3 + k];
    float a = 0.0f, b = 0.0f;
    if (cl != 0u && ch != 0u) { a = grid_decode(~cl); b = grid_decode(ch); }
    o[k] = a; m[k] = b;
  }
  const float tiny = 1e-6f;
  const float ex = (m[0] - o[0]) + tiny, ey = (m[1] - o[1]) + tiny, ez = (m[2] - o[2]) + tiny;
  const float n = (float)(n_tgt > 0 ? n_tgt : 1);
  const float area = ex * ey + ey * ez + ex * ez;
  float c = 1.5f * sqrtf(area / n);
  const float cv = 0.5f * cbrtf((ex * ey * ez) / n);
  c = cv > c ? cv : c;
  const float emax = ex > ey ? (ex > ez ? ex : ez) : (ey > ez ? ey : ez);
  c = c > emax * (1.0f / 1024.0f) ? c : emax * (1.0f / 1024.0f);
  c = c > 1e-6f ? c : 1e-6f;
  int nx, ny, nz;
  for (;;) {
    nx = (int)(ex / c) + 1; ny = (int)(ey / c) + 1; nz = (int)(ez / c) + 1;
    if ((double)nx * (double)ny * (double)nz <= (double)cells_cap) break;
    c *= 1.26f;
  }
  GsGrid g;
  g.ox = o[0]; g.oy = o[1]; g.oz = o[2];
  g.mx = m[0]; g.my = m[1]; g.mz = m[2];
  g.c = c; g.inv_c = 1.0f / c;
  g.nx = nx; g.ny = ny; g.nz = nz; g.ncell = nx * ny * nz;
  return g;
}

GS_DEV void grid_count_body(const float* __restrict__ tgt, const int64_t n_tgt, const GsTargetFilter flt,
                            const unsigned* __restrict__ bbox, GsGrid* __restrict__ gp, int* __restrict__ cell_count,
                            int* __restrict__ tile_sums, int cells_cap, const float4* __restrict__ tlist,
                            const unsigned blk, const unsigned nblk) {
  __shared__ GsGrid gsh;
  __shared__ int th[GS_GRID_MAXCELL / GS_GRID_TILE + 1];
  const int64_t n_items = flt.pix ? (int64_t)bbox[6] : n_tgt;
  if ((int64_t)blk * 256 >= n_items && blk != 0) return;
  if (threadIdx.x == 0) {
    gsh = grid_from_bbox(bbox, n_items, cells_cap);
    if (blk == 0) *gp = gsh;
  }
  __syncthreads();
  const GsGrid g = gsh;
  const int ntile = g.ncell / GS_GRID_TILE + 1;
  for (int t = threadIdx.x; t < ntile; t += 256) th[t] = 0;
  __syncthreads();
  if (flt.pix) {
    for (int64_t i = (int64_t)blk * 256 + threadIdx.x; i < n_items; i += (int64_t)nblk * 256) {
      const float4 t = tlist[i];
      const int cid = grid_cell(g, t.x, t.y, t.z);
      atomicAdd(&cell_count[cid], 1);
      atomicAdd(&th[cid / GS_GRID_TILE], 1);
    }
  } else {
    const int64_t i = (int64_t)blk * 256 + threadIdx.x;
    if (i < n_tgt) {
      const int cid = grid_cell(g, tgt[3 * i], tgt[3 * i + 1], tgt[3 * i + 2]);
      atomicAdd(&cell_count[cid], 1);
      atomicAdd(&th[cid / GS_GRID_TILE], 1);
    }
  }
  __syncthreads();
  for (int t = threadIdx.x; t < ntile; t += 256) {
    const int v = th[t];
    if (v) atomicAdd(&tile_sums[t], v);
  }
}
__global__ void __launch_bounds__(256) gs_grid_count_kernel(const float* __restrict__ tgt, GsCount n_tgt_c,
                                                            const GsTargetFilter flt,
                                                            const unsigned* __restrict__ bbox,
                                                            GsGrid* __restrict__ gp,
                                                            int* __restrict__ cell_count, int* __restrict__ tile_sums,
                                                            int cells_cap, const float4* __restrict__ tlist) {
  grid_count_body(tgt, gs_count(n_tgt_c), flt, bbox, gp, cell_count, tile_sums, cells_cap, tlist, blockIdx.x, gridDim.x);
}

GS_DEV void grid_scan_body(const int* __restrict__ cell_count, const GsGrid* __restrict__ gp,
                           const int* __restrict__ tile_sums, int* __restrict__ cell_start, const unsigned blk) {
  __shared__ int smem[256 / GS_WAVE + 1];
  const int n = gp->ncell + 1;
  if ((int)(blk * GS_GRID_TILE) >= n) return;
  int pre = 0;
  for (int t = threadIdx.x; t < (int)blk; t += 256) pre += tile_sums[t];
  int tile_prefix;
  (void)gs_block_excl_scan<256>(pre, smem, &tile_prefix);
  const int base = blk * GS_GRID_TILE + threadIdx.x * 4;
  int v[4], c = 0;
#pragma unroll
  for (int i = 0; i < 4; ++i) {
    v[i] = (base + i < n) ? cell_count[base + i] : 0;
    c += v[i];
  }
  int total;
  int run = tile_prefix + gs_block_excl_scan<256>(c, smem, &total);
#pragma unroll
  for (int i = 0; i < 4; ++i) {
    if (base + i < n) cell_start[base + i] = run;
    run += v[i];
  }
}
__global__ void __launch_bounds__(256) gs_grid_scan_kernel(const int* __restrict__ cell_count,
                                                           const GsGrid* __restrict__ gp,
                                                           const int* __restrict__ tile_sums,
                                                           int* __restrict__ cell_start) {
  grid_scan_body(cell_count, gp, tile_sums, cell_start, blockIdx.x);
}

GS_DEV void grid_scatter_body(const float* __restrict__ tgt, const int64_t n_tgt, const GsTargetFilter flt,
                              const GsGrid* __restrict__ gp, const int* __restrict__ cell_start,
                              int* __restrict__ cell_count, float4* __restrict__ sorted,
                              const float4* __restrict__ tlist, const unsigned* __restrict__ bbox,
                              const float* __restrict__ nrm, float4* __restrict__ sorted_n, const unsigned blk,
                              const unsigned nblk) {
  if (flt.pix) {
    const int64_t n_list = (int64_t)bbox[6];
    if ((int64_t)blk * 256 >= n_list) return;
    const GsGrid g = *gp;
    for (int64_t i = (int64_t)blk * 256 + threadIdx.x; i < n_list; i += (int64_t)nblk * 256) {
      const float4 t = tlist[i];
      const int cid = grid_cell(g, t.x, t.y, t.z);
      const int slot = cell_start[cid] + atomicSub(&cell_count[cid], 1) - 1;
      sorted[slot] = t;
      if (nrm) {
        const int64_t r = (int64_t)__float_as_int(t.w);
        sorted_n[slot] = make_float4(nrm[3 * r], nrm[3 * r + 1], nrm[3 * r + 2], 0.0f);
      }
    }
    return;
  }
  const int64_t i = (int64_t)blk * 256 + threadIdx.x;
  if (i >= n_tgt) return;
  const GsGrid g = *gp;
  const float x = tgt[3 * i], y = tgt[3 * i + 1], z = tgt[3 * i + 2];
  const int cid = grid_cell(g, x, y, z);
  const int slot = cell_start[cid] + atomicSub(&cell_count[cid], 1) - 1;
  sorted[slot] = make_float4(x, y, z, __int_as_float((int)i));
  if (nrm) sorted_n[slot] = make_float4(nrm[3 * i], nrm[3 * i + 1], nrm[3 * i + 2], 0.0f);
}
__global__ void __launch_bounds__(256) gs_grid_scatter_kernel(const float* __restrict__ tgt, GsCount n_tgt_c,
                                                              const GsTargetFilter flt,
                                                              const GsGrid* __restrict__ gp,
                                                              const int* __restrict__ cell_start,
                                                              int* __restrict__ cell_count,
                                                              float4* __restrict__ sorted,
                                                              const float4* __restrict__ tlist,
                                                              const unsigned* __restrict__ bbox,
                                                              const float* __restrict__ nrm,
                                                              float4* __restrict__ sorted_n) {
  grid_scatter_body(tgt, gs_count(n_tgt_c), flt, gp, cell_start, cell_count, sorted, tlist, bbox, nrm, sorted_n, blockIdx.x,
                    gridDim.x);
}

__global__ void __launch_bounds__(GB_BLOCK) gs_gridb_bbox_kernel(const GsGridBatch gb, float u_hi, float v_hi) {
  gridb_bbox_block(gb, blockIdx.x, u_hi, v_hi);
}
__global__ void __launch_bounds__(256) gs_gridb_count_kernel(const GsGridBatch gb) {
  const GsGridSeq& q = gb.s[blockIdx.x % gb.B];
  grid_count_body(q.tgt, gs_count(q.n_tgt), GsTargetFilter{q.pix, gb.W, gb.ds}, q.m.bbox, q.m.g, q.m.cell_count,
                  q.m.tile_sums, gb.cells_cap, q.m.tlist, blockIdx.x / gb.B, gridDim.x / gb.B);
}
__global__ void __launch_bounds__(256) gs_gridb_scan_kernel(const GsGridBatch gb) {
  const GsGridSeq& q = gb.s[blockIdx.x % gb.B];
  grid_scan_body(q.m.cell_count, q.m.g, q.m.tile_sums, q.m.cell_start, blockIdx.x / gb.B);
}
__global__ void __launch_bounds__(256) gs_gridb_scatter_kernel(const GsGridBatch gb) {
  const GsGridSeq& q = gb.s[blockIdx.x % gb.B];
  grid_scatter_body(q.tgt, gs_count(q.n_tgt), GsTargetFilter{q.pix, gb.W, gb.ds}, q.m.g, q.m.cell_start, q.m.cell_count,
                    q.m.sorted, q.m.tlist, q.m.bbox, q.nrm, q.m.sorted_n, blockIdx.x / gb.B, gridDim.x / gb.B);
}

static int grid_cells_cap(int64_t n_src, int64_t n_tgt_exact) {
  int64_t want = 48 * n_src;
  if (16 * n_tgt_exact > want) want = 16 * n_tgt_exact;
  int cells_cap = 1 << 20;
  while (cells_cap < GS_GRID_MAXCELL && cells_cap < want) cells_cap <<= 1;
  return cells_cap;
}
int gs_knn_grid_cells_cap(int64_t n_src) { return grid_cells_cap(n_src, 0); }
size_t gs_knn_grid_clear_bytes(const GridMem& m, int cells_cap) {
  return gs_align((size_t)(reinterpret_cast<char*>(m.cell_count) - reinterpret_cast<char*>(m.g)) +
                  4 * (size_t)(cells_cap + 1));
}

int gs_knn_grid_build_batch(const GsGridBatch& gb, hipStream_t st, bool bbox_done) {
  int64_t n_max = 1;
  for (int b = 0; b < gb.B; ++b) n_max = gb.s[b].n_tgt.host > n_max ? gb.s[b].n_tgt.host : n_max;
  const unsigned B = (unsigned)gb.B;
  const float u_hi = (float)((double)gb.W - 0.999), v_hi = (float)((double)gb.H - 0.999);
  if (!bbox_done)
    hipLaunchKernelGGL(gs_gridb_bbox_kernel, dim3(gs_knn_gridb_bbox_blocks(gb)), dim3(GB_BLOCK), 0, st, gb, u_hi, v_hi);
  bool listed = true;
  for (int b = 0; b < gb.B; ++b) listed = listed && gb.s[b].pix != nullptr;
  const int64_t slots = (int64_t)gs_ceil_div(gb.H, gb.ds) * gs_ceil_div(gb.W, gb.ds);
  unsigned nb_pts = (unsigned)gs_ceil_div(n_max, 256);
  if (listed && gb.H > 0 && (unsigned)gs_ceil_div(3 * slots, 256) < nb_pts) nb_pts = (unsigned)gs_ceil_div(3 * slots, 256);
  hipLaunchKernelGGL(gs_gridb_count_kernel, dim3(B * nb_pts), dim3(256), 0, st, gb);
  const unsigned ntile = (unsigned)gs_ceil_div(gb.cells_cap + 1, GS_GRID_TILE);
  hipLaunchKernelGGL(gs_gridb_scan_kernel, dim3(B * ntile), dim3(256), 0, st, gb);
  hipLaunchKernelGGL(gs_gridb_scatter_kernel, dim3(B * nb_pts), dim3(256), 0, st, gb);
  hipError_t e = hipGetLastError();
  if (e != hipSuccess) { gs_set_error("gs_knn_grid_build_batch: %s", hipGetErrorString(e)); return GS_ERR_HIP; }
  return GS_OK;
}

int gs_knn_grid_build(const float* tgt, GsCount n_tgt_c, int64_t n_src, void* grid_scratch, hipStream_t st,
                      GsTargetFilter flt, const float* nrm) {
  const int64_t n_tgt = n_tgt_c.host;
  GridMem m = grid_carve(grid_scratch, n_src, n_tgt);
  const int cells_cap = grid_cells_cap(n_src, n_tgt_c.dev ? 0 : n_tgt);
  GsProf prof(GS_PROF_COMPACT, 28.0 * (double)n_tgt + 8.0 * (double)cells_cap, st);
  const size_t clear = gs_knn_grid_clear_bytes(m, cells_cap);
  hipError_t e = hipMemsetAsync(m.g, 0, clear, st);
  if (e != hipSuccess) { gs_set_error("gs_knn_grid_build: %s", hipGetErrorString(e)); return GS_ERR_HIP; }
  hipLaunchKernelGGL(gs_grid_bbox_kernel, dim3((unsigned)gs_ceil_div(n_tgt > 0 ? n_tgt : 1, GB_BLOCK * GB_ITEMS)),
                     dim3(GB_BLOCK), 0, st, tgt, n_tgt_c, flt, m.bbox, m.unres_count, m.tlist);
  hipLaunchKernelGGL(gs_grid_count_kernel, dim3((unsigned)gs_ceil_div(n_tgt > 0 ? n_tgt : 1, 256)), dim3(256), 0, st,
                     tgt, n_tgt_c, flt, m.bbox, m.g, m.cell_count, m.tile_sums, cells_cap, m.tlist);
  const unsigned ntile = (unsigned)gs_ceil_div(cells_cap + 1, GS_GRID_TILE);
  hipLaunchKernelGGL(gs_grid_scan_kernel, dim3(ntile), dim3(256), 0, st, m.cell_count, m.g, m.tile_sums,
                     m.cell_start);
  hipLaunchKernelGGL(gs_grid_scatter_kernel, dim3((unsigned)gs_ceil_div(n_tgt, 256)), dim3(256), 0, st, tgt,
                     n_tgt_c, flt, m.g, m.cell_start, m.cell_count, m.sorted, m.tlist, m.bbox, nrm, m.sorted_n);
  return GS_OK;
}

constexpr int GQ_BLOCK = 256;

__global__ void __launch_bounds__(GQ_BLOCK) gs_grid_query_kernel(
    const float* __restrict__ src_in, const float* __restrict__ Tapply, float* __restrict__ src_out,
    int64_t n_src, const GsGrid* __restrict__ gp, const int* __restrict__ cell_start,
    const float4* __restrict__ sorted, unsigned long long* __restrict__ best, int* __restrict__ unres_count,
    int* __restrict__ unres_next, int* __restrict__ unres_list) {
  const int lane = threadIdx.x & (GQ_G - 1);
  const int64_t s = ((int64_t)blockIdx.x * GQ_BLOCK + threadIdx.x) / GQ_G;
  if (blockIdx.x == 0 && threadIdx.x == 0) *unres_next = 0;
  if (s >= n_src) return;
  const GsGrid g = *gp;
  float qx = src_in[3 * s], qy = src_in[3 * s + 1], qz = src_in[3 * s + 2];
  if (Tapply) {
    float T[12];
#pragma unroll
    for (int i = 0; i < 12; ++i) T[i] = Tapply[i];
    float t0, t1, t2;
    gs_rigid_fma(T, qx, qy, qz, t0, t1, t2);
    qx = t0; qy = t1; qz = t2;
  }
  if (src_out && lane == 0) {
    src_out[3 * s] = qx;
    src_out[3 * s + 1] = qy;
    src_out[3 * s + 2] = qz;
  }
  bool done;
  const unsigned long long key = grid_search_group(g, cell_start, sorted, qx, qy, qz, lane, &done);
  if (lane == 0) {
    if (done) {
      best[s] = key;
    } else {
      best[s] = ~0ull;
      unres_list[atomicAdd(unres_count, 1)] = (int)s;
    }
  }
}

int gs_knn_grid_query(const float* src_in, const float* Tapply, float* src_out, int64_t n_src,
                      const float* tgt, int64_t n_tgt, unsigned long long* best, void* grid_scratch,
                      hipStream_t st) {
  static unsigned seq = 0;
  GridMem m = grid_carve(grid_scratch, n_src, n_tgt);
  int* cnt = m.unres_count + (seq & 1);
  int* nxt = m.unres_count + ((seq + 1) & 1);
  ++seq;
  GsProf prof(GS_PROF_KNN, (double)n_src * (double)n_tgt, st);
  hipLaunchKernelGGL(gs_grid_query_kernel, dim3((unsigned)gs_ceil_div(n_src * GQ_G, GQ_BLOCK)), dim3(GQ_BLOCK), 0, st,
                     src_in, Tapply, src_out, n_src, m.g, m.cell_start, m.sorted, best, cnt, nxt, m.unres_list);
  unsigned gx = (unsigned)gs_ceil_div(n_src, KNN_BLOCK * 4);
  gx = gx > 4 ? 4 : gx;
  dim3 grid(gx, (unsigned)gs_ceil_div(n_tgt, KNN_TCHUNK));
  hipLaunchKernelGGL((gs_knn1_kernel<true, 4>), grid, dim3(KNN_BLOCK), 0, st, src_in, Tapply, nullptr, n_src, tgt,
                     n_tgt, best, m.unres_list, cnt);
  return GS_OK;
}

__global__ void __launch_bounds__(256) gs_knn_unpack_kernel(const unsigned long long* __restrict__ best,
                                                            int64_t n, int64_t n_tgt, int64_t* __restrict__ idx,
                                                            float* __restrict__ d2) {
  const int64_t i = (int64_t)blockIdx.x * 256 + threadIdx.x;
  if (i >= n) return;
  const unsigned long long b = best[i];
  int64_t j = (int64_t)(b & 0xffffffffull);
  if (j >= n_tgt) j = 0;
  idx[i] = j;
  if (d2) d2[i] = __uint_as_float((uint32_t)(b >> 32));
}

extern "C" int gs_knn1_f32(const float* src, int64_t n_src, const float* tgt, int64_t n_tgt,
                           int64_t* out_idx, float* out_d2, uint64_t* best_scratch, void* stream) {
  GS_REQUIRE(n_src > 0 && n_tgt > 0, "empty point set");
  GS_REQUIRE(n_tgt < 0x7fffffffll && n_src < 0x7fffffffll, "too many points");
  GS_REQUIRE(src && tgt && out_idx && best_scratch, "NULL pointer");
  hipStream_t st = gs_stream(stream);
  GS_HIP(hipMemsetAsync(best_scratch, 0xff, 8 * (size_t)n_src, st));
  gs_knn_brute_launch(src, nullptr, nullptr, n_src, tgt, n_tgt, reinterpret_cast<unsigned long long*>(best_scratch), st);
  hipLaunchKernelGGL(gs_knn_unpack_kernel, dim3((unsigned)gs_ceil_div(n_src, 256)), dim3(256), 0, st,
                     reinterpret_cast<const unsigned long long*>(best_scratch), n_src, n_tgt, out_idx, out_d2);
  GS_LAUNCH_CHECK();
  return GS_OK;
}

extern "C" int64_t gs_knn1_grid_scratch_bytes(int64_t n_src, int64_t n_tgt) {
  return (int64_t)(gs_align(8 * (size_t)(n_src > 0 ? n_src : 1)) + gs_knn_grid_scratch_bytes(n_src, n_tgt));
}

extern "C" int gs_knn1_grid_f32(const float* src, int64_t n_src, const float* tgt, int64_t n_tgt,
                                int64_t* out_idx, float* out_d2, void* scratch, int64_t* unresolved_out,
                                void* stream) {
  GS_REQUIRE(n_src > 0 && n_tgt > 0, "empty point set");
  GS_REQUIRE(n_tgt < 0x7fffffffll && n_src < 0x7fffffffll, "too many points");
  GS_REQUIRE(src && tgt && out_idx && scratch, "NULL pointer");
  hipStream_t st = gs_stream(stream);
  unsigned long long* best = reinterpret_cast<unsigned long long*>(scratch);
  void* gscratch = reinterpret_cast<char*>(scratch) + gs_align(8 * (size_t)n_src);
  GS_HIP(hipMemsetAsync(best, 0xff, 8 * (size_t)n_src, st));
  int rc = gs_knn_grid_build(tgt, GsCount{n_tgt, nullptr}, n_src, gscratch, st);
  if (rc != GS_OK) return rc;
  GridMem m = grid_carve(gscratch, n_src, n_tgt);
  rc = gs_knn_grid_query(src, nullptr, nullptr, n_src, tgt, n_tgt, best, gscratch, st);
  if (rc != GS_OK) return rc;
  hipLaunchKernelGGL(gs_knn_unpack_kernel, dim3((unsigned)gs_ceil_div(n_src, 256)), dim3(256), 0, st, best, n_src,
                     n_tgt, out_idx, out_d2);
  if (unresolved_out) {
    int h[2] = {0, 0};
    GS_HIP(hipMemcpyAsync(h, m.unres_count, 8, hipMemcpyDeviceToHost, st));
    GS_HIP(hipStreamSynchronize(st));
    *unresolved_out = (int64_t)h[0] + (int64_t)h[1];
  }
  GS_LAUNCH_CHECK();
  return GS_OK;
}
```

### gradslam_amd/csrc/gs_knn_bbox.h

```cpp
#pragma once
#include "gs_assoc_dev.h"
#include "gs_knn.h"

GS_DEV unsigned grid_code(float v) {
  const unsigned b = __float_as_uint(v);
  return (b & 0x80000000u) ? ~b : (b | 0x80000000u);
}
GS_DEV float grid_decode(unsigned c) {
  return __uint_as_float((c & 0x80000000u) ? (c & 0x7fffffffu) : ~c);
}
constexpr int GB_BLOCK = 256;
constexpr int GB_ITEMS = 8;
GS_DEV void grid_bbox_body(const float* __restrict__ tgt, const int64_t n_tgt, const GsTargetFilter flt,
                           const GsCamera* cam, int H, float u_hi, float v_hi, int32_t* __restrict__ pix_out,
                           unsigned* __restrict__ bbox, int* __restrict__ unres_count, float4* __restrict__ tlist,
                           const unsigned blk) {
  if (blk == 0 && threadIdx.x == 0) { unres_count[0] = 0; unres_count[1] = 0; }
  if ((int64_t)blk * GB_BLOCK * GB_ITEMS >= n_tgt) return;
  __shared__ float red[6][GB_BLOCK / GS_WAVE];
  __shared__ int scan_s[GB_BLOCK / GS_WAVE + 1];
  __shared__ unsigned base_s;
  int hits = 0;
  unsigned hitmask = 0;
  float lo[3] = {3.0e38f, 3.0e38f, 3.0e38f}, hi[3] = {-3.0e38f, -3.0e38f, -3.0e38f};
  const int64_t i0 = (int64_t)blk * GB_ITEMS * GB_BLOCK + threadIdx.x;
  if (cam) {
    float v[GB_ITEMS][3];
#pragma unroll
    for (int u = 0; u < GB_ITEMS; ++u) {
      const int64_t i = i0 + (int64_t)u * GB_BLOCK, ic = i < n_tgt ? i : n_tgt - 1;
      v[u][0] = tgt[3 * ic]; v[u][1] = tgt[3 * ic + 1]; v[u][2] = tgt[3 * ic + 2];
    }
#pragma unroll
    for (int u = 0; u < GB_ITEMS; ++u) {
      const int64_t i = i0 + (int64_t)u * GB_BLOCK;
      if (i < n_tgt) {
        int ph = 0, pw = 0;
        const bool in = gs_project_point_hw(*cam, v[u][0], v[u][1], v[u][2], H, flt.W, u_hi, v_hi, ph, pw);
        pix_out[i] = in ? (int32_t)(ph * flt.W + pw) : -1;
        if (in && gs_on_lattice(ph, pw, flt.ds)) {
          ++hits;
          hitmask |= 1u << u;
#pragma unroll
          for (int k = 0; k < 3; ++k) {
            const float w = v[u][k];
            if (w > -3.0e38f && w < 3.0e38f) {
              lo[k] = w < lo[k] ? w : lo[k];
              hi[k] = w > hi[k] ? w : hi[k];
            }
          }
        }
      }
    }
  } else {
    bool t[GB_ITEMS];
    if (flt.pix) {
      int32_t px[GB_ITEMS];
#pragma unroll
      for (int u = 0; u < GB_ITEMS; ++u) {
        const int64_t i = i0 + (int64_t)u * GB_BLOCK;
        px[u] = flt.pix[i < n_tgt ? i : n_tgt - 1];
      }
#pragma unroll
      for (int u = 0; u < GB_ITEMS; ++u) {
        const int32_t p = px[u];
        t[u] = (i0 + (int64_t)u * GB_BLOCK < n_tgt) && p >= 0 && ((p / flt.W) % flt.ds == 0) && ((p % flt.W) % flt.ds == 0);
      }
    } else {
#pragma unroll
      for (int u = 0; u < GB_ITEMS; ++u) t[u] = i0 + (int64_t)u * GB_BLOCK < n_tgt;
    }
#pragma unroll
    for (int u = 0; u < GB_ITEMS; ++u) {
      if (t[u]) {
        const int64_t i = i0 + (int64_t)u * GB_BLOCK;
        ++hits;
        hitmask |= 1u << u;
#pragma unroll
        for (int k = 0; k < 3; ++k) {
          const float w = tgt[3 * i + k];
          if (w > -3.0e38f && w < 3.0e38f) {
            lo[k] = w < lo[k] ? w : lo[k];
            hi[k] = w > hi[k] ? w : hi[k];
          }
        }
      }
    }
  }
  const int lane = threadIdx.x & 63, wave = threadIdx.x >> 6;
#pragma unroll
  for (int k = 0; k < 3; ++k) {
    float a = lo[k], b = hi[k];
#pragma unroll
    for (int d = 32; d > 0; d >>= 1) {
      const float a2 = __shfl_down(a, d, GS_WAVE), b2 = __shfl_down(b, d, GS_WAVE);
      a = a2 < a ? a2 : a;
      b = b2 > b ? b2 : b;
    }
    if (lane == 0) { red[k][wave] = a; red[3 + k][wave] = b; }
  }
  const bool filtered = flt.pix != nullptr || cam != nullptr;
  __syncthreads();
  if (filtered) {
    int total;
    int pos = gs_block_excl_scan<GB_BLOCK>(hits, scan_s, &total);
    if (threadIdx.x == 0 && total) base_s = atomicAdd(&bbox[6], (unsigned)total);
    __syncthreads();
    if (hitmask) {
      const unsigned base = base_s;
#pragma unroll
      for (int u = 0; u < GB_ITEMS; ++u) {
        if (hitmask & (1u << u)) {
          const int64_t i = ((int64_t)blk * GB_ITEMS + u) * GB_BLOCK + threadIdx.x;
          tlist[base + (unsigned)pos] = make_float4(tgt[3 * i], tgt[3 * i + 1], tgt[3 * i + 2], __int_as_float((int)i));
          ++pos;
        }
      }
    }
  }
  if (threadIdx.x < 3) {
    const int k = threadIdx.x;
    float a = red[k][0], b = red[3 + k][0];
    for (int w = 1; w < GB_BLOCK / GS_WAVE; ++w) {
      a = red[k][w] < a ? red[k][w] : a;
      b = red[3 + k][w] > b ? red[3 + k][w] : b;
    }
    if (a <= b) {
      atomicMax(&bbox[k], ~grid_code(a));
      atomicMax(&bbox[3 + k], grid_code(b));
    }
  }
}

GS_DEV void gridb_bbox_block(const GsGridBatch& gb, const unsigned bid, float u_hi, float v_hi) {
  const GsGridSeq& q = gb.s[bid % gb.B];
  const unsigned blk = bid / gb.B;
  const GsTargetFilter flt{q.pix, gb.W, gb.ds};
  if (q.pose16) {
    const GsCamera cam = gs_camera(q.pose16, q.K16);
    grid_bbox_body(q.tgt, gs_count(q.n_tgt), flt, &cam, gb.H, u_hi, v_hi, q.pix, q.m.bbox, q.m.unres_count, q.m.tlist,
                   blk);
  } else {
    grid_bbox_body(q.tgt, gs_count(q.n_tgt), flt, nullptr, 0, 0.0f, 0.0f, nullptr, q.m.bbox, q.m.unres_count, q.m.tlist,
                   blk);
  }
}
static inline unsigned gs_knn_gridb_bbox_blocks(const GsGridBatch& gb) {
  int64_t n_max = 1;
  for (int b = 0; b < gb.B; ++b) n_max = gb.s[b].n_tgt.host > n_max ? gb.s[b].n_tgt.host : n_max;
  return (unsigned)gb.B * (unsigned)gs_ceil_div(n_max, GB_BLOCK * GB_ITEMS);
}
```

Baseline: 3864.

## Recompute association keys instead of storing per-point keys; drop unused pixel buffer

Removes the per-map-point 64-bit key_pt scratch array; tie settling and merge now recompute the association key from the frame vertex and map point. The merge path also checks the high key word first so it can skip the vertex fetch, and it reuses the fetched vertex for fusion. In localization, the per-point pixel index output is no longer written. A new explicit 'listed' flag replaces inferring listing from the pix pointer. The aim is to save global memory traffic at the cost of extra arithmetic and vertex reads.

```diff
diff --git a/gradslam_amd/csrc/gs_assoc_dev.h b/gradslam_amd/csrc/gs_assoc_dev.h
--- a/gradslam_amd/csrc/gs_assoc_dev.h
+++ b/gradslam_amd/csrc/gs_assoc_dev.h
@@ -97,13 +97,16 @@
   ray = ray + d2 * d2;
   return ((uint64_t)__float_as_uint(inv) << 32) | (uint64_t)__float_as_uint(ray);
 }
-GS_DEV uint64_t gs_assoc_key_v(const float* __restrict__ points, const float* __restrict__ ccounts, const float* f,
-                               int64_t n) {
-  const float inv = 1.0f / (ccounts[n] + 1e-20f);
+GS_DEV uint32_t gs_assoc_key_hi(const float cc) { return __float_as_uint(1.0f / (cc + 1e-20f)); }
+GS_DEV uint32_t gs_assoc_key_lo_v(const float* __restrict__ points, const float* f, int64_t n) {
   const float d0 = points[3 * n] - f[0];
   const float d1 = points[3 * n + 1] - f[1];
   const float d2 = points[3 * n + 2] - f[2];
   float ray = d0 * d0 + d1 * d1;
   ray = ray + d2 * d2;
-  return ((uint64_t)__float_as_uint(inv) << 32) | (uint64_t)__float_as_uint(ray);
+  return __float_as_uint(ray);
 }
+GS_DEV uint64_t gs_assoc_key_v(const float* __restrict__ points, const float* __restrict__ ccounts, const float* f,
+                               int64_t n) {
+  return ((uint64_t)gs_assoc_key_hi(ccounts[n]) << 32) | (uint64_t)gs_assoc_key_lo_v(points, f, n);
+}
diff --git a/gradslam_amd/csrc/gs_fuse.hip b/gradslam_amd/csrc/gs_fuse.hip
--- a/gradslam_amd/csrc/gs_fuse.hip
+++ b/gradslam_amd/csrc/gs_fuse.hip
@@ -85,12 +85,12 @@
   return f;
 }
 
-template <class Frame>
+template <bool HAVE_VERTEX = false, class Frame>
 GS_DEV void fuse_merge_row(float* __restrict__ points, float* __restrict__ normals, float* __restrict__ colors,
                            float* __restrict__ ccounts, const int64_t n, const int32_t p, const Frame& frame,
-                           const float* __restrict__ rgb, const float* __restrict__ alpha) {
+                           const float* __restrict__ rgb, const float* __restrict__ alpha, const float cc,
+                           const float* fv = nullptr) {
   const float a = p >= 0 ? alpha[p] : 0.0f;
-  const float cc = ccounts[n];
   float P[3], N[3], C[3], fp[3] = {0.0f, 0.0f, 0.0f}, fn[3] = {0.0f, 0.0f, 0.0f}, fc[3] = {0.0f, 0.0f, 0.0f};
 #pragma unroll
   for (int k = 0; k < 3; ++k) {
@@ -99,7 +99,13 @@
     C[k] = colors[3 * n + k];
   }
   if (p >= 0) {
-    frame((int64_t)p, fp, fn);
+    if (HAVE_VERTEX) {
+      frame.normal_of((int64_t)p, fn);
+#pragma unroll
+      for (int k = 0; k < 3; ++k) fp[k] = fv[k];
+    } else {
+      frame((int64_t)p, fp, fn);
+    }
 #pragma unroll
     for (int k = 0; k < 3; ++k) fc[k] = rgb[3 * (int64_t)p + k];
   }
@@ -131,7 +137,7 @@
   if (*any_flag == 0 && renorm_all != 2) return;
   const int32_t p = pix_of[n];
   if (p < 0 && !renorm_all) return;
-  fuse_merge_row(points, normals, colors, ccounts, n, p, FrameGlobalMaps{gvertex, gnormal}, rgb, alpha);
+  fuse_merge_row(points, normals, colors, ccounts, n, p, FrameGlobalMaps{gvertex, gnormal}, rgb, alpha, ccounts[n]);
 }
 
 struct PredNewPixel {
@@ -383,7 +389,6 @@
   int32_t* any_flag;
   uint64_t* key_pix;
   int32_t* tile_counts;
-  uint64_t* key_pt;
   int32_t* pix;
   int32_t* pix_of;
 };
@@ -438,7 +443,6 @@
         q.best_pix[p] = MU_TIE_MARK;
         q.any_flag[1] = 1;
       }
-      q.key_pt[n] = k;
       pk = p;
     }
   }
@@ -451,7 +455,10 @@
   for (int64_t n = (int64_t)blk * GS_CP_BLOCK + threadIdx.x; n < n_map; n += (int64_t)nblk * GS_CP_BLOCK) {
     const int32_t p = q.pix[n];
     if (p < 0 || q.best_pix[p] == -1) continue;
-    if (q.key_pt[n] == q.key_pix[p]) atomicMin(reinterpret_cast<unsigned*>(&q.best_pix[p]), (unsigned)n);
+    float fp[3];
+    if (q.gvertex) FrameGlobalMaps{q.gvertex, q.gnormal}.vertex_of((int64_t)p, fp);
+    else frame_local_maps(q.vertex, q.normal, q.pose16).vertex_of((int64_t)p, fp);
+    if (gs_assoc_key_v(q.points, q.ccounts, fp, n) == q.key_pix[p]) atomicMin(reinterpret_cast<unsigned*>(&q.best_pix[p]), (unsigned)n);
   }
 }
 
@@ -489,24 +496,33 @@
   mu_settle_ties(q, blk, gridDim.x / mb.B);
 }
 
+template <class Frame>
+GS_DEV void mu_merge_row(const MuBatch& mb, const MuSeq& q, const int64_t n, const Frame& frame) {
+  int32_t p = q.pix[n];
+  const float cc = q.ccounts[n];
+  float fp[3] = {0.0f, 0.0f, 0.0f};
+  if (p >= 0) {
+    const uint64_t kp = q.key_pix[p];
+    bool win = (uint32_t)(kp >> 32) == gs_assoc_key_hi(cc);
+    if (win) {
+      frame.vertex_of((int64_t)p, fp);
+      const int32_t bp = q.best_pix[p];
+      win = (uint32_t)kp == gs_assoc_key_lo_v(q.points, fp, n) && (bp == -1 || bp == (int32_t)n);
+      if (win && bp == -1) q.best_pix[p] = (int32_t)n;
+    }
+    if (!win) p = -1;
+  }
+  if (p < 0 && !mb.renorm_all) return;
+  fuse_merge_row<true>(q.points, q.normals, q.colors, q.ccounts, n, p, frame, q.rgb, q.alpha, cc, fp);
+}
+
 GS_DEV void mu_merge_body(const MuBatch& mb, const unsigned bid) {
   const MuSeq& q = mb.s[bid % mb.B];
   const int64_t n = (int64_t)(bid / mb.B) * 256 + threadIdx.x;
   if (n >= gs_count(q.n_map)) return;
   if (*mb.call_flag == 0) return;
-  int32_t p = q.pix[n];
-  if (p >= 0) {
-    bool win = q.key_pt[n] == q.key_pix[p];
-    if (win) {
-      const int32_t bp = q.best_pix[p];
-      win = bp == -1 || bp == (int32_t)n;
-      if (win && bp == -1) q.best_pix[p] = (int32_t)n;
-    }
-    if (!win) p = -1;
-  }
-  if (p < 0 && !mb.renorm_all) return;
-  if (q.gvertex) fuse_merge_row(q.points, q.normals, q.colors, q.ccounts, n, p, FrameGlobalMaps{q.gvertex, q.gnormal}, q.rgb, q.alpha);
-  else fuse_merge_row(q.points, q.normals, q.colors, q.ccounts, n, p, frame_local_maps(q.vertex, q.normal, q.pose16), q.rgb, q.alpha);
+  if (q.gvertex) mu_merge_row(mb, q, n, FrameGlobalMaps{q.gvertex, q.gnormal});
+  else mu_merge_row(mb, q, n, frame_local_maps(q.vertex, q.normal, q.pose16));
 }
 
 GS_DEV void mu_append_body(const MuBatch& mb, const unsigned bid) {
@@ -575,7 +591,6 @@
 extern "C" int64_t gs_update_map_scratch_bytes(int64_t n_map_bound, int H, int W) {
   const int64_t P = (int64_t)H * W;
   return (int64_t)(256 + gs_align(8 * (size_t)P) + gs_align(4 * (size_t)gs_cp_tiles(P)) +
-                   gs_align(8 * (size_t)(n_map_bound > 0 ? n_map_bound : 1)) +
                    2 * gs_align(4 * (size_t)(n_map_bound > 0 ? n_map_bound : 1)) + 4096);
 }
 
@@ -611,11 +626,10 @@
     m.any_flag = reinterpret_cast<int32_t*>(q); q += 256;
     m.key_pix = reinterpret_cast<uint64_t*>(q); q += gs_align(8 * (size_t)mb.P);
     m.tile_counts = reinterpret_cast<int32_t*>(q); q += gs_align(4 * (size_t)mb.ntiles);
-    m.key_pt = reinterpret_cast<uint64_t*>(q); q += gs_align(8 * (size_t)(n_map > 0 ? n_map : 1));
     m.pix = reinterpret_cast<int32_t*>(q); q += gs_align(4 * (size_t)(n_map > 0 ? n_map : 1));
     m.pix_of = reinterpret_cast<int32_t*>(q);
-    bytes_assoc += 72.0 * (double)n_map;
-    bytes_fuse += 104.0 * (double)n_map + 49.0 * (double)mb.P;
+    bytes_assoc += 64.0 * (double)n_map;
+    bytes_fuse += 96.0 * (double)n_map + 49.0 * (double)mb.P;
   }
   const unsigned uB = (unsigned)B;
   const unsigned pb = uB * (unsigned)gs_ceil_div(mb.P, 256), nb = uB * (unsigned)gs_ceil_div(n_max > 0 ? n_max : 1, 256);
diff --git a/gradslam_amd/csrc/gs_icp_loop.hip b/gradslam_amd/csrc/gs_icp_loop.hip
--- a/gradslam_amd/csrc/gs_icp_loop.hip
+++ b/gradslam_amd/csrc/gs_icp_loop.hip
@@ -1199,14 +1199,13 @@
 struct LocLayout {
   int64_t n_lat, rows;
   IcpLayout sc;
-  size_t lattice, pix, n_valid, icp, lq, ls, lstat, far_c, far_cq, far_idx, far_n, far_out4, total;
+  size_t lattice, n_valid, icp, lq, ls, lstat, far_c, far_cq, far_idx, far_n, far_out4, total;
 };
 static LocLayout loc_layout(int64_t n_lat, int64_t rows) {
   GsTake take;
   LocLayout L;
   L.n_lat = n_lat; L.rows = rows > 0 ? rows : 1;
   L.lattice = take(gs_align(12 * (size_t)n_lat));
-  L.pix = take(gs_align(4 * (size_t)L.rows));
   L.n_valid = take(256);
   L.sc = icp_layout(n_lat, L.rows);
   L.icp = take(L.sc.total);
@@ -1230,13 +1229,13 @@
 }
 
 struct LocCarve {
-  float* lattice; int32_t* pix; int64_t* n_valid;
+  float* lattice; int64_t* n_valid;
   IcpScratch sc; GridMem gm; ListMem lm;
   FarMem fm; int* far_out4;
 };
 static LocCarve loc_carve(void* p, const LocLayout& L) {
   const IcpScratch sc = icp_carve(gs_at<char>(p, L.icp), L.sc);
-  return LocCarve{gs_at<float>(p, L.lattice), gs_at<int32_t>(p, L.pix), gs_at<int64_t>(p, L.n_valid), sc,
+  return LocCarve{gs_at<float>(p, L.lattice), gs_at<int64_t>(p, L.n_valid), sc,
                   grid_carve(sc.grid, L.n_lat, L.rows),
                   ListMem{gs_at<float4>(p, L.lq), gs_at<uint32_t>(p, L.ls), gs_at<int>(p, L.lstat)},
                   FarMem{gs_at<uint32_t>(p, L.far_c), gs_at<float4>(p, L.far_cq), gs_at<int>(p, L.far_idx), gs_at<int>(p, L.far_n)},
@@ -1302,6 +1301,7 @@
 static void loc_bind(const gs_localize_seq* seqs, int B, int H, int W, int ds, const gs_icp_params* prm,
                      const IcpEnginePlan& plan, LocCarve* c, LocBatch& lb, GsGridBatch& gb, IcpSolveView* v) {
   lb.B = gb.B = B; lb.W = gb.W = W; gb.H = H; lb.ds = gb.ds = ds;
+  gb.listed = 1;
   lb.Wl = (W + ds - 1) / ds; lb.n_lat = loc_lattice(H, W, ds); lb.damp = prm->damp; lb.numiters = prm->numiters;
   gb.cells_cap = gs_knn_grid_cells_cap(lb.n_lat);
   for (int b = 0; b < B; ++b) {
@@ -1310,7 +1310,7 @@
     lb.s[b] = LocSeq{q.vertex, q.depth, q.prev_pose16, c[b].lattice, c[b].sc.state, q.out_pose16,
                      reinterpret_cast<char*>(c[b].gm.g), c[b].n_valid, c[b].fm.n, c[b].lm.stat,
                      plan.wide_on ? c[b].fm.cq : nullptr, c[b].sc.sync};
-    gb.s[b] = GsGridSeq{q.map.points, GsCount{q.map.n_bound, q.map.n_dev}, c[b].pix, q.prev_pose16, q.K16,
+    gb.s[b] = GsGridSeq{q.map.points, GsCount{q.map.n_bound, q.map.n_dev}, nullptr, q.prev_pose16, q.K16,
                         plan.binned_normals ? q.map.normals : nullptr, c[b].gm};
     v[b] = IcpSolveView{c[b].lattice, q.map.points, q.map.normals, GsCount{q.map.n_bound, q.map.n_dev}, c[b].sc, c[b].gm,
                         nullptr, TapePtrs{nullptr, nullptr, nullptr},
@@ -1331,7 +1331,7 @@
   const unsigned nb_lat = (unsigned)gs_ceil_div(lb.n_lat, 256);
   const unsigned nb_clear = (unsigned)gs_ceil_div((int64_t)(lb.clear_bytes / 16), 256 * LP_CLEAR_ITEMS);
   double bytes = 0.0;
-  for (int b = 0; b < B; ++b) bytes += 28.0 * lb.n_lat + 24.0 * seqs[b].map.n_bound + 16.0 * gb.cells_cap;
+  for (int b = 0; b < B; ++b) bytes += 28.0 * lb.n_lat + 12.0 * seqs[b].map.n_bound + 16.0 * gb.cells_cap;
   GsProf prof(GS_PROF_COMPACT, bytes, st, grid_cleared ? 4 : 5);
   if (grid_cleared) {
     const float u_hi = (float)((double)gb.W - 0.999), v_hi = (float)((double)gb.H - 0.999);
@@ -1453,7 +1453,7 @@
                    int64_t n_tgt, const float* init16, const float* compose16,
                    const gs_icp_params* prm, float* out_T16, int64_t* out_idx, void* icp_scratch,
                    void* tape, void* stream, const int64_t* n_src_dev = nullptr,
-                   const int64_t* n_tgt_dev = nullptr, GsTargetFilter flt = GsTargetFilter{nullptr, 1, 1}) {
+                   const int64_t* n_tgt_dev = nullptr, GsTargetFilter flt = GsTargetFilter{nullptr, 1, 1, 0}) {
   GS_REQUIRE(prm, "params_host must not be NULL");
   GS_REQUIRE(n_src > 0 && n_tgt > 0, "empty point set");
   GS_REQUIRE(n_tgt < 0x7fffffffll && n_src < 0x7fffffffll, "too many points");
@@ -1463,7 +1463,7 @@
   IcpScratch sc = icp_carve(icp_scratch, icp_layout(n_src, n_tgt));
   hipLaunchKernelGGL(gs_icp_init_kernel, dim3(1), dim3(64), 0, st, sc.state, init16, prm->damp, prm->numiters,
                      compose16, out_T16);
-  const bool dev_counts = n_src_dev || n_tgt_dev || flt.pix;
+  const bool dev_counts = n_src_dev || n_tgt_dev || flt.listed;
   const bool use_grid = prm->numiters > 0 && (dev_counts || (!gs_env().knn_brute && gs_knn_use_grid(n_src, n_tgt)));
   const GsCount n_src_c{n_src, n_src_dev}, n_tgt_c{n_tgt, n_tgt_dev};
   TapePtrs tp = {nullptr, nullptr, nullptr};
@@ -1483,7 +1483,7 @@
     double prof_bytes = 0.0;
     if (g_gs_prof_on) {
       int64_t n_binned = n_tgt;
-      if (flt.pix) {
+      if (flt.listed) {
         unsigned hits = 0;
         GS_HIP(hipMemcpyAsync(&hits, v.gm.bbox + 6, 4, hipMemcpyDeviceToHost, st));
         GS_HIP(hipStreamSynchronize(st));
@@ -1560,7 +1560,7 @@
                                  void* icp_scratch, void* stream) {
   GS_REQUIRE(pix && W > 0 && ds > 0, "bad target filter");
   return icp_run(src, n_src_bound, map_points, map_normals, n_map_bound, init16, compose16, prm, out_T16, nullptr,
-                 icp_scratch, nullptr, stream, n_src_dev, n_map_dev, GsTargetFilter{pix, W, ds});
+                 icp_scratch, nullptr, stream, n_src_dev, n_map_dev, GsTargetFilter{pix, W, ds, 1});
 }
 
 static int localize_chunk(const gs_localize_seq* seqs, int B, int H, int W, int ds, const gs_icp_params* prm,
diff --git a/gradslam_amd/csrc/gs_knn.h b/gradslam_amd/csrc/gs_knn.h
--- a/gradslam_amd/csrc/gs_knn.h
+++ b/gradslam_amd/csrc/gs_knn.h
@@ -22,6 +22,7 @@
 struct GsTargetFilter {
   const int32_t* pix;
   int W, ds;
+  int listed;
 };
 GS_DEV bool gs_is_target(const GsTargetFilter& f, int64_t n) {
   if (!f.pix) return true;
@@ -72,6 +73,7 @@
 };
 struct GsGridBatch {
   int B, H, W, ds;
+  int listed;
   int cells_cap;
   GsGridSeq s[GS_MAX_BATCH];
 };
@@ -80,7 +82,7 @@
 int gs_knn_grid_build_batch(const GsGridBatch& gb, hipStream_t st, bool bbox_done = false);
 
 int gs_knn_grid_build(const float* tgt, GsCount n_tgt, int64_t n_src, void* grid_scratch, hipStream_t st,
-                      GsTargetFilter filter = GsTargetFilter{nullptr, 1, 1}, const float* nrm = nullptr);
+                      GsTargetFilter filter = GsTargetFilter{nullptr, 1, 1, 0}, const float* nrm = nullptr);
 int gs_knn_grid_query(const float* src_in, const float* Tapply, float* src_out, int64_t n_src,
                       const float* tgt, int64_t n_tgt, unsigned long long* best, void* grid_scratch,
                       hipStream_t st);
diff --git a/gradslam_amd/csrc/gs_knn.hip b/gradslam_amd/csrc/gs_knn.hip
--- a/gradslam_amd/csrc/gs_knn.hip
+++ b/gradslam_amd/csrc/gs_knn.hip
@@ -151,7 +151,7 @@
                             const unsigned blk, const unsigned nblk) {
   __shared__ GsGrid gsh;
   __shared__ int th[GS_GRID_MAXCELL / GS_GRID_TILE + 1];
-  const int64_t n_items = flt.pix ? (int64_t)bbox[6] : n_tgt;
+  const int64_t n_items = flt.listed ? (int64_t)bbox[6] : n_tgt;
   if ((int64_t)blk * 256 >= n_items && blk != 0) return;
   if (threadIdx.x == 0) {
     gsh = grid_from_bbox(bbox, n_items, cells_cap);
@@ -162,7 +162,7 @@
   const int ntile = g.ncell / GS_GRID_TILE + 1;
   for (int t = threadIdx.x; t < ntile; t += 256) th[t] = 0;
   __syncthreads();
-  if (flt.pix) {
+  if (flt.listed) {
     for (int64_t i = (int64_t)blk * 256 + threadIdx.x; i < n_items; i += (int64_t)nblk * 256) {
       const float4 t = tlist[i];
       const int cid = grid_cell(g, t.x, t.y, t.z);
@@ -229,7 +229,7 @@
                               const float4* __restrict__ tlist, const unsigned* __restrict__ bbox,
                               const float* __restrict__ nrm, float4* __restrict__ sorted_n, const unsigned blk,
                               const unsigned nblk) {
-  if (flt.pix) {
+  if (flt.listed) {
     const int64_t n_list = (int64_t)bbox[6];
     if ((int64_t)blk * 256 >= n_list) return;
     const GsGrid g = *gp;
@@ -273,7 +273,7 @@
 }
 __global__ void __launch_bounds__(256) gs_gridb_count_kernel(const GsGridBatch gb) {
   const GsGridSeq& q = gb.s[blockIdx.x % gb.B];
-  grid_count_body(q.tgt, gs_count(q.n_tgt), GsTargetFilter{q.pix, gb.W, gb.ds}, q.m.bbox, q.m.g, q.m.cell_count,
+  grid_count_body(q.tgt, gs_count(q.n_tgt), GsTargetFilter{q.pix, gb.W, gb.ds, gb.listed}, q.m.bbox, q.m.g, q.m.cell_count,
                   q.m.tile_sums, gb.cells_cap, q.m.tlist, blockIdx.x / gb.B, gridDim.x / gb.B);
 }
 __global__ void __launch_bounds__(256) gs_gridb_scan_kernel(const GsGridBatch gb) {
@@ -282,7 +282,7 @@
 }
 __global__ void __launch_bounds__(256) gs_gridb_scatter_kernel(const GsGridBatch gb) {
   const GsGridSeq& q = gb.s[blockIdx.x % gb.B];
-  grid_scatter_body(q.tgt, gs_count(q.n_tgt), GsTargetFilter{q.pix, gb.W, gb.ds}, q.m.g, q.m.cell_start, q.m.cell_count,
+  grid_scatter_body(q.tgt, gs_count(q.n_tgt), GsTargetFilter{q.pix, gb.W, gb.ds, gb.listed}, q.m.g, q.m.cell_start, q.m.cell_count,
                     q.m.sorted, q.m.tlist, q.m.bbox, q.nrm, q.m.sorted_n, blockIdx.x / gb.B, gridDim.x / gb.B);
 }
 
@@ -306,8 +306,7 @@
   const float u_hi = (float)((double)gb.W - 0.999), v_hi = (float)((double)gb.H - 0.999);
   if (!bbox_done)
     hipLaunchKernelGGL(gs_gridb_bbox_kernel, dim3(gs_knn_gridb_bbox_blocks(gb)), dim3(GB_BLOCK), 0, st, gb, u_hi, v_hi);
-  bool listed = true;
-  for (int b = 0; b < gb.B; ++b) listed = listed && gb.s[b].pix != nullptr;
+  const bool listed = gb.listed != 0;
   const int64_t slots = (int64_t)gs_ceil_div(gb.H, gb.ds) * gs_ceil_div(gb.W, gb.ds);
   unsigned nb_pts = (unsigned)gs_ceil_div(n_max, 256);
   if (listed && gb.H > 0 && (unsigned)gs_ceil_div(3 * slots, 256) < nb_pts) nb_pts = (unsigned)gs_ceil_div(3 * slots, 256);
diff --git a/gradslam_amd/csrc/gs_knn_bbox.h b/gradslam_amd/csrc/gs_knn_bbox.h
--- a/gradslam_amd/csrc/gs_knn_bbox.h
+++ b/gradslam_amd/csrc/gs_knn_bbox.h
@@ -37,7 +37,7 @@
       if (i < n_tgt) {
         int ph = 0, pw = 0;
         const bool in = gs_project_point_hw(*cam, v[u][0], v[u][1], v[u][2], H, flt.W, u_hi, v_hi, ph, pw);
-        pix_out[i] = in ? (int32_t)(ph * flt.W + pw) : -1;
+        if (pix_out) pix_out[i] = in ? (int32_t)(ph * flt.W + pw) : -1;
         if (in && gs_on_lattice(ph, pw, flt.ds)) {
           ++hits;
           hitmask |= 1u << u;
@@ -99,9 +99,8 @@
     }
     if (lane == 0) { red[k][wave] = a; red[3 + k][wave] = b; }
   }
-  const bool filtered = flt.pix != nullptr || cam != nullptr;
   __syncthreads();
-  if (filtered) {
+  if (flt.listed) {
     int total;
     int pos = gs_block_excl_scan<GB_BLOCK>(hits, scan_s, &total);
     if (threadIdx.x == 0 && total) base_s = atomicAdd(&bbox[6], (unsigned)total);
@@ -135,7 +134,7 @@
 GS_DEV void gridb_bbox_block(const GsGridBatch& gb, const unsigned bid, float u_hi, float v_hi) {
   const GsGridSeq& q = gb.s[bid % gb.B];
   const unsigned blk = bid / gb.B;
-  const GsTargetFilter flt{q.pix, gb.W, gb.ds};
+  const GsTargetFilter flt{q.pix, gb.W, gb.ds, gb.listed};
   if (q.pose16) {
     const GsCamera cam = gs_camera(q.pose16, q.K16);
     grid_bbox_body(q.tgt, gs_count(q.n_tgt), flt, &cam, gb.H, u_hi, v_hi, q.pix, q.m.bbox, q.m.unres_count, q.m.tlist,
```

Result: faster. 3972 (median of 6 runs) (+2.8%).
